# VladimirP1/rs-sync

Hardware: AMD Instinct MI355X
Metric: ray-residuals/sec (PreSync sweep + Sync iter), 4096 frames x 2048 tracks (higher is better)
Workload: dtype f32

## Files before the change

rs-sync_amd/csrc/kernels/support.hpp:

```cpp
#pragma once

namespace {

__global__ __launch_bounds__(64) void plan_sum_kernel(const double* __restrict__ in, uint32_t n_cols,
                                                         const uint32_t* __restrict__ idx,
                                                         const uint32_t* __restrict__ chunk_off, uint32_t n_chunks,
                                                         const uint32_t* __restrict__ win_chunk_off, uint32_t n_win,
                                                         double* __restrict__ chunk_out, double* __restrict__ win_out) {
    const uint32_t r = blockIdx.x / n_win, w = blockIdx.x % n_win;
    const uint32_t c0 = win_chunk_off[w], c1 = win_chunk_off[w + 1];
    const double* row = in + (size_t)r * n_cols;
    double* cout = chunk_out + (size_t)r * n_chunks;
    for (uint32_t c = c0 + threadIdx.x; c < c1; c += blockDim.x) {
        double acc = 0.0;
        uint32_t j = chunk_off[c];
        const uint32_t j1 = chunk_off[c + 1];
        for (; j + 8 <= j1; j += 8) {
            double v[8];
#pragma unroll
            for (int q = 0; q < 8; ++q) v[q] = row[idx ? idx[j + q] : j + q];
#pragma unroll
            for (int q = 0; q < 8; ++q) acc += v[q];
        }
        for (; j < j1; ++j) acc += row[idx ? idx[j] : j];
        cout[c] = acc;
    }
    __syncthreads();
    if (threadIdx.x == 0) {
        double acc = 0.0;
        uint32_t c = c0;
        for (; c + 16 <= c1; c += 16) {
            double v[16];
#pragma unroll
            for (int q = 0; q < 16; ++q) v[q] = cout[c + q];
#pragma unroll
            for (int q = 0; q < 16; ++q) acc += v[q];
        }
        for (; c < c1; ++c) acc += cout[c];
        win_out[blockIdx.x] = acc;
    }
}

struct DebugParams {
    const f4* rays_a;
    const f4* rays_b;
    const FrameRec* frames;
    uint32_t fi;
    const f4* coef;
    int n_knots;
    float fs;
    int32_t kd;
    float fd;
    float* P;
    float* dP;
};

__global__ __launch_bounds__(kBlock) void debug_problem_kernel(DebugParams p) {
    __shared__ f4 s_win[4 * kWinMax];
    const FrameRec fr = p.frames[p.fi];
    Spline sp;
    sp.g = p.coef;
    sp.n = p.n_knots;
    stage_window(sp, s_win, fr.base_knot + (int)floorf(fr.tmin) + p.kd, fr.base_knot + (int)floorf(fr.tmax) + p.kd + 1);
    __syncthreads();
    for (uint32_t row = blockIdx.x * kBlock + threadIdx.x; row < fr.n; row += gridDim.x * kBlock) {
        f3 P, dP;
        if (sp.path == kPathInterior) residual_row<true, kPathInterior>(sp, p.rays_a[fr.off + row], p.rays_b[fr.off + row], fr.base_knot + p.kd, p.fd, P, dP);
        else residual_row<true, kPathGlobal>(sp, p.rays_a[fr.off + row], p.rays_b[fr.off + row], fr.base_knot + p.kd, p.fd, P, dP);
        p.P[3 * row] = P.x; p.P[3 * row + 1] = P.y; p.P[3 * row + 2] = P.z;
        if (p.dP) { p.dP[3 * row] = dP.x * p.fs; p.dP[3 * row + 1] = dP.y * p.fs; p.dP[3 * row + 2] = dP.z * p.fs; }
    }
}

struct PackParams {
    const double* raw;
    const rship_pack_frame* frames;
    f4* rays_a;
    f4* rays_b;
    double2* q0;
    double2* q1;
    double2* q2;
    double2* q3;
    double start, fs;
    uint32_t* bad;
};

__device__ __forceinline__ double pixel_knot_offset(double ro, double py, double frame_time, double rows, double start, double fs,
                                                   double base) {
    return rs::knot_offset(rs::row_time(ro, py, frame_time, rows), start, fs, base);
}

__global__ __launch_bounds__(kBlock) void pack_frames_kernel(PackParams p) {
    const rship_pack_frame& fr = p.frames[blockIdx.x];
    const uint32_t n = fr.n_rays;
    for (uint32_t row = blockIdx.y * kBlock + threadIdx.x; row < n; row += gridDim.y * kBlock) {
        double ra[3], rb[3], tsa, tsb, ta, tb;
        const double* rec = p.raw + fr.raw_offset;
        if (fr.is_pixels) {
            const double2* src = (const double2*)(rec + 4 * (size_t)row);
            const double2 a = src[0], b = src[1];
            const rs::Lens lens{fr.lens[0], fr.lens[1], fr.lens[2], fr.lens[3], fr.lens[4], fr.lens[5], fr.lens[6], fr.lens[7], fr.lens[8]};
            rs::pixel_to_ray(lens, a.x, a.y, fr.time_a, fr.rows, ra, &tsa);
            rs::pixel_to_ray(lens, b.x, b.y, fr.time_b, fr.rows, rb, &tsb);
            ta = pixel_knot_offset(lens.ro, a.y, fr.time_a, fr.rows, p.start, p.fs, fr.base);
            tb = pixel_knot_offset(lens.ro, b.y, fr.time_b, fr.rows, p.start, p.fs, fr.base);
        } else {
            tsa = rec[row];
            tsb = rec[(size_t)n + row];
            const double* pa = rec + 2 * (size_t)n + 3 * (size_t)row;
            const double* pb = rec + 5 * (size_t)n + 3 * (size_t)row;
            ra[0] = pa[0]; ra[1] = pa[1]; ra[2] = pa[2];
            rb[0] = pb[0]; rb[1] = pb[1]; rb[2] = pb[2];
            ta = rs::knot_offset(tsa, p.start, p.fs, fr.base);
            tb = rs::knot_offset(tsb, p.start, p.fs, fr.base);
        }
        f4 o0, o1;
        o0.x = (float)ra[0]; o0.y = (float)rb[0]; o0.z = (float)ra[1]; o0.w = (float)rb[1];
        o1.x = (float)ra[2]; o1.y = (float)rb[2]; o1.z = (float)ta; o1.w = (float)tb;
        const bool ok = finite_f(o0.x) && finite_f(o0.y) && finite_f(o0.z) && finite_f(o0.w) && finite_f(o1.x) &&
                        finite_f(o1.y) && finite_f(o1.z) && finite_f(o1.w);
        if (!ok) atomicAdd(p.bad, 1u);
        const size_t o = (size_t)fr.ray_offset + row;
        p.rays_a[o] = o0;
        p.rays_b[o] = o1;
        p.q0[o] = double2{ra[0], rb[0]};
        p.q1[o] = double2{ra[1], rb[1]};
        p.q2[o] = double2{ra[2], rb[2]};
        p.q3[o] = double2{ta, tb};
    }
}

struct RetimeParams {
    const double* raw;
    const rship_pack_frame* pack;
    const FrameRec* frames;
    const double* ro;
    f4* rays_b;
    double2* q3;
    double start, fs;
};

__global__ __launch_bounds__(kBlock) void retime_pixels_kernel(RetimeParams p) {
    const rship_pack_frame& fr = p.pack[blockIdx.x];
    if (!fr.is_pixels) return;
    const uint32_t n = fr.n_rays;
    const double ro = p.ro[blockIdx.x], base = (double)p.frames[blockIdx.x].base_knot;
    const double* rec = p.raw + fr.raw_offset;
    for (uint32_t row = blockIdx.y * kBlock + threadIdx.x; row < n; row += gridDim.y * kBlock) {
        const double ya = rec[4 * (size_t)row + 1], yb = rec[4 * (size_t)row + 3];
        const double ta = pixel_knot_offset(ro, ya, fr.time_a, fr.rows, p.start, p.fs, base);
        const double tb = pixel_knot_offset(ro, yb, fr.time_b, fr.rows, p.start, p.fs, base);
        const size_t o = (size_t)fr.ray_offset + row;
        ((float2*)(p.rays_b + o))[1] = make_float2((float)ta, (float)tb);
        p.q3[o] = double2{ta, tb};
    }
}

__global__ __launch_bounds__(64) void debug_select_kernel(const float* __restrict__ vals, uint32_t n, uint32_t kq,
                                                          const float* __restrict__ upper, uint32_t* out) {
    constexpr int NR = 32;
    const int lane = threadIdx.x;
    const float* v = vals + (size_t)blockIdx.x * n;
// ... 27 lines not shown
```

rs-sync_amd/csrc/kernels/sync64.hpp:

```cpp
#pragma once

#pragma clang fp contract(off)

namespace {



struct Loss64Params {
    Rays64 rays;
    const FrameRec* frames;
    const uint32_t* sel;
    uint32_t n_sel;
    const d4* coef;
    int n_knots;
    double fs;
    const int32_t* kd;
    const double* fd;
    uint32_t n_delays;
    const uint32_t* grp;
    uint32_t n_grp;
    const double* M;
    const double* k;
    double* part_loss;
    double* part_grad;
// ... 392 lines not shown
    if (fd != fd) {
        if (tid == 0 && p.evals_out) p.evals_out[sf] = 0;
        if (mk_out) { mk_out[0] = m_x; mk_out[1] = m_y; mk_out[2] = m_z; mk_out[3] = m_k; }
        return;
    }

    Spline64 sp;
    sp.g = p.coef;
    sp.n = p.n_knots;
    sp.cap = (int)p.win_cap;
    sp.compact = (int)p.win_compact;
    frame_window64(sp, s_win, fr, kd);
    __syncthreads();

    MotionEval64<RPT, NW, EMU4> ev;
    ev.part = s_part;
    ev.buf = 0;
    ev.evals = 0;
    const int base = fr.base_knot + kd;
    ev.gP = nullptr;
    ev.g_rows = 0;
    ev.rpt = RPT;
    if constexpr (RPT != 0) {
#pragma unroll
        for (int j = 0; j < RPT; ++j) {
            const uint32_t row = j * kThreads + tid;
            d3 P = d3{0, 0, 0}, dP;
            if (row < N) residual_row64<false>(sp, p.rays, (size_t)fr.off + row, base, fd, P, dP);
            ev.P[j] = P;
        }
    } else {
        double* gp = p.scratch + (size_t)scratch_entry * 3 * p.scratch_rows;
        ev.gP = gp;
        ev.g_rows = p.scratch_rows;
        constexpr int kGroup = EMU4 ? 256 : kThreads;
        ev.rpt = (int)((N + kGroup - 1) / kGroup);
        for (uint32_t row = tid; row < (uint32_t)ev.rpt * kGroup; row += kThreads) {
            d3 P = d3{0, 0, 0}, dP;
            if (row < N) residual_row64<false>(sp, p.rays, (size_t)fr.off + row, base, fd, P, dP);
            gp[row] = P.x; gp[p.scratch_rows + row] = P.y; gp[2 * (size_t)p.scratch_rows + row] = P.z;
        }
    }

    double x[3];
    double kk;
    if (p.simple_k || pend != kInitNone) {
        d3 Mv = d3{0, 0, 0};
        if (!p.simple_k && pend >= 0) {
            uint32_t i0, i1;
            rs::sample_pair(p.seed, fr.id, p.win_stream ? ld_m<SC1>(&p.win_stream[grp]) : p.stream_base + grp * p.stream_stride, (uint32_t)pend, N, i0, i1);
            d3 P0, P1, dP;
            residual_row64<false>(sp, p.rays, (size_t)fr.off + i0, base, fd, P0, dP);
            residual_row64<false>(sp, p.rays, (size_t)fr.off + i1, base, fd, P1, dP);
            Mv = rs::cross(P0, P1);
            const double nn = sqrt(rs::dot(Mv, Mv));
            if (!(nn < 1e-12)) Mv = rs::scale(Mv, 1.0 / nn);
        }
        double tot;
        if constexpr (EMU4) {
            tot = 0.0;
            for (int vw = 0; vw < 4; ++vw) {
                double ss = 0.0;
                for (int j = 0; j < ev.rpt; ++j) {
                    const size_t i = (size_t)j * 256 + (size_t)vw * 64 + tid;
                    const d3 Pj = d3{ev.gP[i], ev.gP[ev.g_rows + i], ev.gP[2 * (size_t)ev.g_rows + i]};
                    const double pm = p.simple_k ? sqrt(rs::dot(Pj, Pj)) : rs::dot(Pj, Mv);
                    ss = fma(pm, pm, ss);
                }
                const double sw = wave_sum_f64(ss);
                tot = vw == 0 ? sw : tot + sw;
            }
        } else {
        double ss = 0.0;
        if constexpr (RPT != 0) {
#pragma unroll
            for (int j = 0; j < RPT; ++j) {
                const double pm = p.simple_k ? sqrt(rs::dot(ev.P[j], ev.P[j])) : rs::dot(ev.P[j], Mv);
                ss = fma(pm, pm, ss);
            }
        } else {
            for (int j = 0; j < ev.rpt; ++j) {
                const size_t i = (size_t)j * kThreads + tid;
                const d3 Pj = d3{ev.gP[i], ev.gP[ev.g_rows + i], ev.gP[2 * (size_t)ev.g_rows + i]};
                const double pm = p.simple_k ? sqrt(rs::dot(Pj, Pj)) : rs::dot(Pj, Mv);
                ss = fma(pm, pm, ss);
            }
        }
        const double sw = wave_sum_f64(ss);
        if ((tid & 63) == 0) s_red[tid >> 6] = sw;
        __syncthreads();
        tot = s_red[0];
#pragma unroll
        for (int w = 1; w < NW; ++w) tot += s_red[w];
        }
        kk = clamp_k(100.0 / sqrt(tot));
        x[0] = Mv.x; x[1] = Mv.y; x[2] = Mv.z;
        if (tid == 0) {
            if (!p.simple_k) { st_m<SC1>(&p.M[3 * sf], x[0]); st_m<SC1>(&p.M[3 * sf + 1], x[1]); st_m<SC1>(&p.M[3 * sf + 2], x[2]); }
            st_m<SC1>(&p.k[sf], kk);
            if (p.init_h) st_m<SC1>(&p.init_h[sf], (int32_t)kInitNone);
        }
    } else {
        x[0] = m_x; x[1] = m_y; x[2] = m_z;
        kk = m_k;
    }
    if (mk_out) { mk_out[0] = x[0]; mk_out[1] = x[1]; mk_out[2] = x[2]; mk_out[3] = kk; }
    if (p.max_iters <= 0 || p.simple_k) return;
    ev.k2 = kk * kk;
    if constexpr (EMU4) {
        if ((size_t)N * 24u <= (size_t)p.win_bytes) {
            __syncthreads();
            __attribute__((address_space(3))) double* l = (__attribute__((address_space(3))) double*)reinterpret_cast<double*>(s_win);
            for (uint32_t row = tid; row < N; row += kThreads) {
                l[row] = ev.gP[row];
                l[N + row] = ev.gP[ev.g_rows + row];
                l[2 * N + row] = ev.gP[2 * (size_t)ev.g_rows + row];
            }
            __syncthreads();
            ev.lP = l;
            ev.n_lds = N;
        }
    }

    LbfgsHistLds hist{s_S, s_Y, s_inv_ys, s_rho, s_alpha};
    int best_not_last = 0;
    K3_T0();
    const int it = rs::lbfgs3(ev, hist, x, p.max_iters , p.reeval, &best_not_last);
    K3_ADD(12, 13);
    K3_FLUSH(ev);
    if (mk_out) { mk_out[0] = x[0]; mk_out[1] = x[1]; mk_out[2] = x[2]; }
    if (tid == 0) {
        st_m<SC1>(&p.M[3 * sf], x[0]); st_m<SC1>(&p.M[3 * sf + 1], x[1]); st_m<SC1>(&p.M[3 * sf + 2], x[2]);
        if (p.stats) {
            atomicAdd(&p.stats[0], (unsigned long long)it);
            atomicAdd(&p.stats[1], (unsigned long long)ev.evals);
            atomicAdd(&p.stats[2], (unsigned long long)best_not_last);
        }
        if (p.per_frame) {
            p.per_frame[2 * sf] = (uint32_t)it;
            p.per_frame[2 * sf + 1] = (uint32_t)ev.evals;
        }
        if (p.evals_out) p.evals_out[sf] = (uint32_t)ev.evals;
    }
}

template <int RPT, int NW>
__global__ __launch_bounds__(64 * NW, NW == 4 ? (RPT == 0 ? 2 : (RPT <= 8 ? 3 : (RPT <= 24 ? 2 : 1))) : (NW == 1 ? (RPT >= 8 ? 3 : 4) : 2)) void opt_motion64_kernel(Motion64Params p) {
    __shared__ MotionLds<NW> lds;
    extern __shared__ d4 s_motion_win[];
    opt_motion64_body<RPT, NW>(p, p.order ? p.order[blockIdx.x + p.slot0] : blockIdx.x + p.slot0, lds, s_motion_win, nullptr,
                               p.scratch0 + blockIdx.x);
}

__global__ __launch_bounds__(1024) void motion_order_kernel(const uint32_t* __restrict__ evals, const uint32_t* __restrict__ list,
                                                            uint32_t* __restrict__ order, uint32_t pos0, uint32_t count) {
    __shared__ uint32_t s_bin[256];
    for (uint32_t b = threadIdx.x; b < 256; b += blockDim.x) s_bin[b] = 0;
    __syncthreads();
    for (uint32_t i = threadIdx.x; i < count; i += blockDim.x) {
        const uint32_t e = evals[list[pos0 + i]];
        atomicAdd(&s_bin[e < 255u ? e : 255u], 1u);
    }
    __syncthreads();
    if (threadIdx.x == 0) {
        uint32_t at = 0;
        for (int b = 255; b >= 0; --b) {
            const uint32_t n = s_bin[b];
            s_bin[b] = at;
            at += n;
        }
    }
    __syncthreads();
    for (uint32_t i = threadIdx.x; i < count; i += blockDim.x) {
        const uint32_t s = list[pos0 + i];
        const uint32_t e = evals[s];
        const uint32_t pos = atomicAdd(&s_bin[e < 255u ? e : 255u], 1u);
        order[pos0 + pos] = s;
    }
}

struct Debug64Params {
    Rays64 rays;
    const FrameRec* frames;
    uint32_t fi;
    const d4* coef;
    int n_knots;
    double fs;
    int32_t kd;
    double fd;
    double* P;
    double* dP;
};

__global__ __launch_bounds__(kBlock) void debug_problem64_kernel(Debug64Params p) {
    __shared__ d4 s_win[4 * kWinMax];
    const FrameRec fr = p.frames[p.fi];
    Spline64 sp;
    sp.g = p.coef;
    sp.n = p.n_knots;
    sp.cap = kWinMax;
    sp.compact = 0;
    frame_window64(sp, s_win, fr, p.kd);
    __syncthreads();
    for (uint32_t row = blockIdx.x * kBlock + threadIdx.x; row < fr.n; row += gridDim.x * kBlock) {
        d3 P, dP;
        residual_row64<true>(sp, p.rays, (size_t)fr.off + row, fr.base_knot + p.kd, p.fd, P, dP);
        p.P[3 * row] = P.x; p.P[3 * row + 1] = P.y; p.P[3 * row + 2] = P.z;
        if (p.dP) { p.dP[3 * row] = dP.x * p.fs; p.dP[3 * row + 1] = dP.y * p.fs; p.dP[3 * row + 2] = dP.z * p.fs; }
    }
}

__global__ __launch_bounds__(64) void debug_math64_kernel(int op, const double* __restrict__ a, const double* __restrict__ b,
                                                          double* __restrict__ out, uint32_t n) {
    const uint32_t i = blockIdx.x * 64 + threadIdx.x;
    const double x = i < n ? a[i] : 0.0, y = (i < n && b) ? b[i] : 0.0;
    if (op == 4) {
        const double t = wave_sum_f64(x);
        if (threadIdx.x == 0) out[blockIdx.x] = t;
        return;
    }
    if (i >= n) return;
    if (op == 0) out[i] = x / y;
    else if (op == 1) out[i] = sqrt(x);
    else if (op == 2) { double rc; out[2 * i] = rs::log1p_rcp_f64(x, &rc); out[2 * i + 1] = rc; }
    else if (op == 5) out[i] = rs::div3_exact(x);
    else out[i] = fma(x, y, x);
}

}

#pragma clang fp contract(fast)
```

rs-sync_amd/csrc/kernels/syncloop.hpp:

```cpp
#pragma once

namespace {

constexpr int kMaxBt = 10, kHalfBt = 5;

struct SyncWin {
    double d, v;
    double x0;
    double l1, g1;
    int active, conv, hit, iters;
    int phase;
    int nf;
    int hit_prev;
};

struct SyncLoopParams {
    SyncWin* win;
    uint32_t n_win;
    uint32_t win0, win1;
    const double* part;
    uint32_t n_sel, rows;
    const uint32_t* chunk_off;
    const uint32_t* win_chunk_off;
    double* chunk_tmp;
    uint32_t chunk_stride;
    int32_t* mo_kd; double* mo_fd;
    int32_t* lg_kd; double* lg_fd;
    int32_t* tr_kd; double* tr_fd;
    double fs;
    double ts[11];
    double c_armijo, delay_b, search_center, search_radius;
    int it, max_outer;
    int nf_fixed;
    int nf_floor;
    double* ext_sums;
    int* n_active;
    double* trace;
};


__device__ __forceinline__ void split64_dev(double delay, double fs, int32_t* kd, double* fd) {
#pragma clang fp contract(off)
    if (delay != delay) { *kd = 0; *fd = delay; return; }
    const double D = delay * fs;
    const double kClamp = (double)(1 << 29);
    if (!(fabs(D) <= 1.79769313486231570e308)) { *kd = 0; *fd = 0.0; return; }
    const double fl = floor(D);
    if (fl > kClamp) { *kd = 1 << 29; *fd = 0.0; return; }
    if (fl < -kClamp) { *kd = -(1 << 29); *fd = 0.0; return; }
    *kd = (int32_t)fl;
    *fd = D - fl;
}

constexpr uint32_t kStageDoubles = 2048;
__device__ __forceinline__ void window_sums(const SyncLoopParams& p, uint32_t w, double* s_tot, double* s_stage) {
    const uint32_t c0 = p.win_chunk_off[w], c1 = p.win_chunk_off[w + 1], nc = c1 - c0;
    const uint32_t j_lo = p.chunk_off[c0], j_hi = p.chunk_off[c1], span = j_hi - j_lo;
    double* tmp = p.chunk_tmp + (size_t)w * (2 * kMaxBt) * p.chunk_stride;
    const bool staged = p.rows * span <= kStageDoubles;
    if (staged) {
        for (uint32_t e = threadIdx.x; e < p.rows * span; e += blockDim.x)
            s_stage[e] = p.part[(size_t)(e / span) * p.n_sel + j_lo + e % span];
        __syncthreads();
    }
    for (uint32_t e = threadIdx.x; e < p.rows * nc; e += blockDim.x) {
        const uint32_t r = e / nc, c = c0 + e % nc;
        double acc = 0.0;
        uint32_t j = p.chunk_off[c];
        const uint32_t j1 = p.chunk_off[c + 1];
        if (staged) {
            const double* row = s_stage + (size_t)r * span - j_lo;
            for (; j + 8 <= j1; j += 8) {
                double v[8];
#pragma unroll
                for (int q = 0; q < 8; ++q) v[q] = row[j + q];
#pragma unroll
                for (int q = 0; q < 8; ++q) acc += v[q];
            }
            for (; j < j1; ++j) acc += row[j];
        } else {
            const double* row = p.part + (size_t)r * p.n_sel;
            const uint32_t cnt = j1 - j;
            if (cnt <= 64) {
                double v[64];
#pragma unroll
                for (int q = 0; q < 64; ++q) v[q] = (uint32_t)q < cnt ? row[j + q] : 0.0;
#pragma unroll
                for (int q = 0; q < 64; ++q)
                    if ((uint32_t)q < cnt) acc += v[q];
            } else {
                for (; j < j1; ++j) acc += row[j];
            }
        }
        tmp[(size_t)r * p.chunk_stride + (c - c0)] = acc;
    }
    __syncthreads();
    for (uint32_t r = threadIdx.x; r < p.rows; r += blockDim.x) {
        const double* t = tmp + (size_t)r * p.chunk_stride;
        double acc = 0.0;
        uint32_t c = 0;
        for (; c + 16 <= nc; c += 16) {
            double v[16];
#pragma unroll
            for (int q = 0; q < 16; ++q) v[q] = t[c + q];
#pragma unroll
            for (int q = 0; q < 16; ++q) acc += v[q];
        }
        for (; c < nc; ++c) acc += t[c];
        s_tot[r] = acc;
    }
    __syncthreads();
}

__global__ __launch_bounds__(64) void sync_begin_kernel(SyncLoopParams p) {
#pragma clang fp contract(off)
    const uint32_t w = p.win0 + blockIdx.x * 64 + threadIdx.x;
    if (w >= p.win1) return;
    SyncWin& s = p.win[w];
    s.x0 = s.active ? s.d - p.delay_b * s.v : __builtin_nan("");
    split64_dev(s.active ? s.d : __builtin_nan(""), p.fs, &p.mo_kd[w], &p.mo_fd[w]);
    split64_dev(s.x0, p.fs, &p.lg_kd[w], &p.lg_fd[w]);
}

__device__ __forceinline__ bool trial_wanted(const SyncWin& s, int i) {
    if (!s.active) return false;
    return s.phase == 0 ? i < s.nf : i >= s.nf;
}

__device__ __forceinline__ void grad_decide(const SyncLoopParams& p, SyncWin& s, double l1, double g1) {
#pragma clang fp contract(off)
    if (s.active && s.phase == 0) {
        s.l1 = l1;
        s.g1 = g1;
        s.hit = -1;
        if (s.iters == 0 && !p.nf_fixed) {
            int i = 0;
            while (i < kMaxBt - 1 && p.ts[i] * fabs(s.g1) >= 1e-3) ++i;
            const int want = i + 2;
            s.nf = want < kHalfBt ? kHalfBt : (want > kMaxBt ? kMaxBt : want);
        }
    }
}
__device__ __forceinline__ void trial_delays(const SyncLoopParams& p, const SyncWin& s, int32_t* tr_kd, double* tr_fd, size_t stride) {
#pragma clang fp contract(off)
    for (int i = 0; i < kMaxBt; ++i) {
        const double td = trial_wanted(s, i) ? s.x0 - p.ts[i] * s.g1 : __builtin_nan("");
        split64_dev(td, p.fs, &tr_kd[(size_t)i * stride], &tr_fd[(size_t)i * stride]);
    }
}

__global__ __launch_bounds__(kBlock) void sync_sums_kernel(SyncLoopParams p) {
#pragma clang fp contract(off)
    __shared__ double s_tot[2 * kMaxBt];
    __shared__ double s_stage[kStageDoubles];
    const uint32_t w = blockIdx.x + p.win0;
    window_sums(p, w, s_tot, s_stage);
    for (uint32_t r = threadIdx.x; r < p.rows; r += blockDim.x) p.ext_sums[(size_t)r * p.n_win + w] = s_tot[r];
}
__device__ __forceinline__ void decision_sums(const SyncLoopParams& p, uint32_t w, double* s_tot, double* s_stage) {
    if (p.ext_sums) {
        for (uint32_t r = threadIdx.x; r < p.rows; r += blockDim.x) s_tot[r] = p.ext_sums[(size_t)r * p.n_win + w];
        __syncthreads();
    } else {
        window_sums(p, w, s_tot, s_stage);
    }
}

__global__ __launch_bounds__(kBlock) void sync_grad_kernel(SyncLoopParams p) {
#pragma clang fp contract(off)
    __shared__ double s_tot[2 * kMaxBt];
    __shared__ double s_stage[kStageDoubles];
    const uint32_t w = blockIdx.x + p.win0;
    decision_sums(p, w, s_tot, s_stage);
    if (threadIdx.x != 0) return;
    SyncWin& s = p.win[w];
    grad_decide(p, s, s_tot[0], s_tot[1]);
    trial_delays(p, s, p.tr_kd + w, p.tr_fd + w, p.n_win);
}

__device__ __forceinline__ void armijo(const SyncLoopParams& p, SyncWin& s, const double* lt, int b0, int b1) {
#pragma clang fp contract(off)
    if (!s.active || s.hit >= 0) return;
    const double m = s.g1 * s.g1;
    for (int i = b0; i < b1; ++i) {
        if (s.l1 - lt[i] >= p.ts[i] * p.c_armijo * m) {
            s.hit = i;
            break;
        }
    }
}

__device__ __forceinline__ bool step_decide(const SyncLoopParams& p, SyncWin& s, const double* lt, double* rows, size_t row_stride) {
#pragma clang fp contract(off)
    bool step_now = false;
    if (s.active) {
        if (s.phase == 0) {
            armijo(p, s, lt, 0, s.nf);
            if (s.hit >= 0 || s.nf >= kMaxBt) step_now = true;
            else s.phase = 1;
        } else {
            armijo(p, s, lt, s.nf, kMaxBt);
            step_now = true;
        }
    }
    if (step_now) {
        const double v = s.l1, g = s.g1;
        const double t = s.hit >= 0 ? p.ts[s.hit] : p.ts[kMaxBt];
        const int trials = s.hit >= 0 ? s.hit + 1 : kMaxBt;
        const double step = -t * g;
        s.v = p.delay_b * s.v + step;
        s.d += s.v;
        const double step_size = fabs(step);
        double* row = rows + (size_t)s.iters * row_stride;
        row[0] = s.d; row[1] = step; row[2] = v; row[3] = g; row[4] = t; row[5] = (double)trials;
        s.iters += 1;
        s.phase = 0;
        const int last = s.hit >= 0 ? s.hit : kMaxBt - 1;
        const int want = (last > s.hit_prev ? last : s.hit_prev) + 1;
        s.hit_prev = last;
        s.nf = p.nf_fixed ? p.nf_fixed : (want < p.nf_floor ? p.nf_floor : (want > kMaxBt ? kMaxBt : want));
        if (step_size < 1e-4) s.conv++; else s.conv = 0;
        bool stop = s.conv > 5;
        if (!stop && fabs(s.d - p.search_center) > p.search_radius) stop = true;
        if (stop || s.iters == p.max_outer) s.active = 0;
    }
    s.x0 = s.active ? s.d - p.delay_b * s.v : __builtin_nan("");
    return step_now;
}

__global__ __launch_bounds__(kBlock) void sync_step_kernel(SyncLoopParams p) {
#pragma clang fp contract(off)
    __shared__ double s_tot[2 * kMaxBt];
    __shared__ double s_stage[kStageDoubles];
    const uint32_t w = blockIdx.x + p.win0;
    decision_sums(p, w, s_tot, s_stage);
    if (threadIdx.x != 0) return;
    SyncWin& s = p.win[w];
    step_decide(p, s, s_tot, p.trace + (size_t)w * 6, (size_t)p.n_win * 6);
    if (s.active) atomicAdd(&p.n_active[p.it], 1);
    const bool go = s.active && s.phase == 0;
    split64_dev(go ? s.d : __builtin_nan(""), p.fs, &p.mo_kd[w], &p.mo_fd[w]);
    split64_dev(go ? s.x0 : __builtin_nan(""), p.fs, &p.lg_kd[w], &p.lg_fd[w]);
}

}
```

rs-sync_amd/csrc/rssync_kernels.hip:

```cpp
#include <hip/hip_runtime.h>

#include <dlfcn.h>

#include <algorithm>
#include <cmath>
#include <cstdio>
#include <cstdlib>
#include <cstring>
#include <mutex>
#include <string>
#include <thread>
#include <vector>

#ifndef RSSYNC_TEST_VARIANTS
#define RSSYNC_TEST_VARIANTS 0
#endif

#include "../../include/rssync_hip.h"
#include "track_hip.h"
#include "rectify_hip.h"
#include "stabilize_hip.h"
#include "color_hip.h"
#include "zoom_hip.h"
#include "limit_hip.h"
#include "colorzoom_hip.h"
#include "infill_hip.h"
#include "colorinfill_hip.h"
#include "device_math.hpp"
#include "sync_math.hpp"
#include "lens_math.hpp"
#include "rectify_math.hpp"
#include "stabilize_math.hpp"
#include "color_math.hpp"
#include "resample_math.hpp"
#include "zoom_math.hpp"
#include "limit_math.hpp"
#include "infill_math.hpp"
#include "gyro_math.hpp"
#include "gyro_signal_math.hpp"
#include "window_plan.hpp"
#include "frame_plan.hpp"
#include "roctx_ranges.hpp"

using rs::f3;
using rs::f4;

#include "kernels/common.hpp"
#include "kernels/rows64.hpp"
#include "kernels/lmeds.hpp"
#include "kernels/lmeds_small.hpp"
#include "kernels/lmeds_big.hpp"
#include "kernels/support.hpp"
#include "kernels/sync64.hpp"
#include "kernels/syncloop.hpp"
#include "kernels/exec_big.hpp"
#include "kernels/executor.hpp"
#include "kernels/gyro.hpp"
#include "kernels/track.hpp"
#include "kernels/features.hpp"
#include "kernels/rectify.hpp"
#include "kernels/stabilize.hpp"
#include "kernels/color.hpp"
#include "kernels/color16.hpp"
#include "kernels/resample.hpp"
#include "kernels/zoom.hpp"
#include "kernels/limit.hpp"
#include "kernels/colorzoom.hpp"
#include "kernels/infill.hpp"
#include "kernels/colorinfill.hpp"


struct DevBuf {
    void* p = nullptr;
    size_t cap = 0;
};
struct TempBuf : DevBuf {
    TempBuf() = default;
    TempBuf(const TempBuf&) = delete;
    TempBuf& operator=(const TempBuf&) = delete;
    ~TempBuf() {
        if (p) (void)hipFree(p);
    }
};

constexpr int kNumClasses = 6;

struct rship_ctx {
    int device = 0;
    hipStream_t own_stream = nullptr;
    hipStream_t stream = nullptr;
    hipStream_t copy_stream = nullptr;
    hipEvent_t copy_done = nullptr;
    std::string err;
    DevBuf coef, coef64, raw, rays_a, rays_b, rays64, frames, sel, M, k, grp, grp_off, init_h;
    DevBuf pack_list, retime_ro;
    std::vector<std::vector<char>> retime_staged;
    std::vector<uint32_t> h_ray_off;
    double pack_start = 0, pack_fs = 0;
    DevBuf mo_evals, mo_order;
    std::vector<std::pair<uint32_t, uint32_t>> mo_ranges;
    bool mo_identity = false;
    DevBuf plan_idx, plan_chunk_off, plan_win_off, chunk_out, win_out;
    uint32_t plan_max_chunks = 0;
    DevBuf g_ts, g_rates, g_us, g_dq, g_q, g_knots, g_cf, g_status;
    uint32_t g_n = 0;
    DevBuf gc_a, gc_b, gc_seg, gc_rates;
    bool gc_on = false;
    uint32_t gc_n = 0, gc_k = 1;
    double gc_sr = 0, gc_first = 0;
    double g_first_s = 0, g_last_s = 0;
    DevBuf trk_slot[2], trk_out;
    DevBuf ftr_cells, ftr_out;
    hipEvent_t trk_up[2] = {}, trk_k[2] = {};
    DevBuf rect_rays, rect_slot[2], rect_times, rect_count, rect_tmp;
    double rect_key[10] = {};
    bool rect_rays_ok = false;
    DevBuf stab_weights, stab_targets, stab_zooms, stab_cover;
    DevBuf rect_rays_c;
    DevBuf limit_goal, limit_out, limit_rays;
    double rect_key_c[10] = {};
    bool rect_rays_c_ok = false;
    int64_t g_first_us = 0, g_last_us = 0;
    std::vector<hipStream_t> loop_streams;
    hipEvent_t loop_ready = nullptr;
    std::vector<uint32_t> h_grp_off;
    DevBuf loop_state;
    bool plan_has_idx = false;
    uint32_t plan_chunks = 0, plan_wins = 0, plan_len = 0;
    struct Pend { uint32_t rows = 0; bool grad = false, frame_costs = false, best_h = false; size_t off_chunk = 0, off_flags = 0; } pend;
    bool init_pending = false;
    uint64_t init_seed = 0;
    uint32_t init_stream = 0, init_stride = 0;
    uint32_t n_knots = 0, n_frames = 0, n_sel = 0, max_n = 0, n_grp = 1;
    uint64_t total_rays = 0;
    double fs = 0;
    int lbfgs_reeval = 0;
    DevBuf cls_slots;
    std::vector<uint32_t> h_cls_slots;
    uint32_t cls_off[kNumClasses + 1] = {};
    uint32_t cls_max_n[kNumClasses] = {};
    int cls_used = 0;
    std::vector<rs::FrameDims> own_dims, problem_dims;
    uint32_t cls_cap64[kNumClasses] = {80, 80, 80, 80, 80, 80};
    bool cls_compact = false;
    bool no_compact = false;
    bool force_general = false;
    uint32_t one_wave_max = 512;
    uint32_t exec_big_max = 2048;
    uint32_t exec_big_share = 8;
    bool force_big = false;
    bool no_small_loss = false;
    bool exact_select = false;
    bool no_subshapes = false;
    bool no_small_lmeds = false;
    float max_span = 0.f;
    float max_ends = 0.f;
    int lds_per_cu = 160 * 1024;
    uint32_t last_lmeds_shape[kNumClasses] = {};
    uint32_t last_lmeds_cap = 0, last_lmeds_chunk = 0, last_init_cap = 0;
    void* rccl_lib = nullptr;
    std::string rccl_path;
    void* rccl_comm = nullptr;
    DevBuf rccl_buf;
    DevBuf big_scratch, mo_scratch;
    rship_loop_exchange_fn loop_xchg = nullptr;
    void* loop_xchg_user = nullptr;
    uint64_t loop_exchanges = 0;
    uint32_t exec_last[4] = {0, 0, 0, 0};
    std::vector<uint32_t> h_frame_n;
    std::vector<uint32_t> h_sel;
    std::vector<uint32_t> h_delays, h_delays64;
    const float* d_fd = nullptr;
    DevBuf kd64;
    const double* d_fd64 = nullptr;
    DevBuf redo_mask, redo_delays, redo_count, init_delays64;
    bool no_fp64_rows = false;
    bool redo_dirty = true;
    uint64_t near_launches = 0;
    struct PendRedo { bool armed = false; LmedsParams p{}; double step_knots = 0; uint32_t chunk = 1; bool uploaded = false; } pend_redo;
    std::vector<int32_t> h_kd64r;
    std::vector<double> h_fd64r;
    std::vector<uint32_t> h_init64;
    uint32_t batch_n = 0, batch_next = 0, batch_rows = 0;
    size_t batch_chunk_stride = 0, batch_win_stride = 0;
    DevBuf dump, dump_ncont;
    bool dump_on = false;
    uint32_t dump_rows = 0, dump_dims[4] = {0, 0, 0, 0}, dump_ncont_n = 0;
    DevBuf kd, frame_cost, best_h, costs, part, flags, stats;
    void* pinned = nullptr;
    size_t pinned_cap = 0;
    bool prof = false;
    struct Pending { int kind; hipEvent_t a, b; };
    std::vector<Pending> pending;
    std::vector<hipEvent_t> pool;
    uint64_t launches[RSHIP_K_COUNT] = {};
    double total_ms[RSHIP_K_COUNT] = {};
};

namespace {

std::mutex g_err_mutex;
int set_err(rship_ctx* c, const char* what, hipError_t e) {
    std::lock_guard<std::mutex> lock(g_err_mutex);
    c->err = std::string(what) + ": " + hipGetErrorString(e);
    return 1;
}
int set_err(rship_ctx* c, const std::string& what) {
    std::lock_guard<std::mutex> lock(g_err_mutex);
    c->err = what;
    return 1;
}

#define RS_HIP(call)                                         \
    do {                                                     \
        hipError_t e__ = (call);                             \
        if (e__ != hipSuccess) return set_err(c, #call, e__); \
    } while (0)

int ensure(rship_ctx* c, DevBuf& b, size_t bytes) {
    if (bytes <= b.cap) return 0;
    if (b.p) RS_HIP(hipFree(b.p));
    b.p = nullptr;
    b.cap = 0;
    size_t want = bytes + bytes / 4 + 256;
    RS_HIP(hipMalloc(&b.p, want));
    b.cap = want;
    return 0;
}

int ensure_pinned(rship_ctx* c, size_t bytes) {
    if (bytes <= c->pinned_cap) return 0;
    if (c->pinned) RS_HIP(hipHostFree(c->pinned));
    c->pinned = nullptr;
    c->pinned_cap = 0;
    size_t want = bytes + bytes / 4 + 4096;
    RS_HIP(hipHostMalloc(&c->pinned, want, hipHostMallocDefault));
    c->pinned_cap = want;
    return 0;
}

const char* const kKindNames[RSHIP_K_COUNT] = {"rssync:K2 lmeds sweep", "rssync:K1 loss (trials)", "rssync:K3 motion L-BFGS", "rssync:window sums",
                                               "rssync:K2 GuessMotion search", "rssync:pack frames", "rssync:gyro pipeline", "rssync:K1 loss+gradient",
                                               "rssync:retime pixels"};
struct ProfScope {
    rship_ctx* c;
    int kind;
    hipEvent_t a = nullptr, b = nullptr;
    rs::RoctxRange range;
    ProfScope(rship_ctx* c_, int kind_) : c(c_), kind(kind_), range(kKindNames[kind_]) {
        if (!c->prof) return;
        auto get = [&]() {
            hipEvent_t e = nullptr;
            if (!c->pool.empty()) { e = c->pool.back(); c->pool.pop_back(); }
            else (void)hipEventCreate(&e);
            return e;
        };
        a = get();
        b = get();
        (void)hipEventRecord(a, c->stream);
    }
    ~ProfScope() {
        if (!c->prof) return;
        (void)hipEventRecord(b, c->stream);
        c->pending.push_back({kind, a, b});
    }
};

void prof_collect(rship_ctx* c) {
    for (auto& pd : c->pending) {
        float ms = 0.f;
        if (hipEventElapsedTime(&ms, pd.a, pd.b) == hipSuccess) {
            c->launches[pd.kind] += 1;
            c->total_ms[pd.kind] += (double)ms;
        }
        c->pool.push_back(pd.a);
        c->pool.push_back(pd.b);
    }
    c->pending.clear();
}

int sync_stream(rship_ctx* c) {
    RS_HIP(hipStreamSynchronize(c->stream));
    prof_collect(c);
    c->retime_staged.clear();
    return 0;
}

constexpr int kMaxRpt = 32;
constexpr int kFourWaveMaxRpt = 24;
constexpr int kWideBlock = 512;

static_assert(rs::kPlanBlock == (uint32_t)kBlock && rs::kPlanFourWaveMaxRpt == (uint32_t)kFourWaveMaxRpt && rs::kPlanMaxRpt == (uint32_t)kMaxRpt,
              "window_plan.hpp (the rules, checked on the CPU by tests/test_window_plan.py) and this file disagree on the size classes");
int class_of(const rship_ctx* c, uint32_t n) {
    if (c->force_big) return 5;
    return rs::plan_class_of(n, c->one_wave_max);
}
void class_bounds(const rship_ctx* c, int k, uint32_t* lo, uint32_t* hi) {
    if (c->force_big) { *lo = k == 5 ? 0u : 1u; *hi = k == 5 ? 0xffffffffu : 0u; return; }
    const uint32_t top[6] = {c->one_wave_max, 4u * kBlock, 8u * kBlock, (uint32_t)kFourWaveMaxRpt * kBlock, (uint32_t)kMaxRpt * kBlock, 0xffffffffu};
    *hi = top[k];
    *lo = k == 0 ? 0u : top[k - 1] + 1u;
}
int class_rpt(const rship_ctx* c, int k) { return rs::plan_class_shape(k, c->cls_max_n[k]); }
int small_rpt(uint32_t n_all) { return rs::plan_small_rows(n_all, false); }
int rpt_for(uint32_t max_n) {
    if (max_n > (uint32_t)kMaxRpt * kBlock) return 0;
    int rpt = 4;
    while ((uint32_t)rpt * kBlock < max_n) rpt *= 2;
    return rpt;
}
uint32_t big_rows(uint32_t max_n) { return (max_n + kBlock - 1) / kBlock * kBlock; }

const std::vector<rs::FrameDims>& plan_dims(const rship_ctx* c) { return c->problem_dims.empty() ? c->own_dims : c->problem_dims; }
void update_class_caps(rship_ctx* c) {
    const std::vector<rs::FrameDims>& d = plan_dims(c);
    for (int k = 0; k < kNumClasses; ++k) {
        uint32_t lo, hi;
        class_bounds(c, k, &lo, &hi);
        bool comp = false;
        const bool may_compact = k == 0 && !c->no_compact && !c->no_small_loss && !c->force_general;
        c->cls_cap64[k] = c->force_general ? (uint32_t)rs::kPlanWinStatic : rs::cap64_frames(d.data(), d.size(), lo, hi, k == 0, may_compact ? &comp : nullptr);
        if (k == 0) c->cls_compact = comp;
    }
}

struct ClassRange {
    int k;
    uint32_t pos0, count;
    const uint32_t* list;
};
std::vector<ClassRange> class_ranges(const rship_ctx* c, uint32_t slot0 = 0, uint32_t count = 0) {
    std::vector<ClassRange> out;
    if (!count) { slot0 = 0; count = c->n_sel; }
    const uint32_t* L = c->h_cls_slots.data();
    for (int k = 0; k < kNumClasses; ++k) {
        const uint32_t* a = L + c->cls_off[k];
        const uint32_t* b = L + c->cls_off[k + 1];
        if (a == b) continue;
        const uint32_t* lo = std::lower_bound(a, b, slot0);
        const uint32_t* hi = std::lower_bound(a, b, slot0 + count);
        if (lo == hi) continue;
        const uint32_t pos0 = (uint32_t)(lo - L);
        out.push_back(ClassRange{k, pos0, (uint32_t)(hi - lo), c->cls_used > 1 ? (const uint32_t*)c->cls_slots.p + pos0 : nullptr});
    }
    return out;
}
int main_class(const rship_ctx* c) {
    int best = 0;
    uint32_t most = 0;
    for (int k = 0; k < kNumClasses; ++k) {
        const uint32_t n = c->cls_off[k + 1] - c->cls_off[k];
        if (n > most) { most = n; best = k; }
    }
    if (!most) {
        uint32_t mx = 0;
        for (const rs::FrameDims& d : c->own_dims) mx = std::max(mx, d.n);
        best = class_of(c, mx);
    }
    return best;
}

constexpr uint32_t kLossWinBytes = kLossBatch * kWinMax * 128u;
using rs::WinPlan;
static_assert(rs::kPlanWinStatic == (uint32_t)kWinMax, "window_plan.hpp and kernels/common.hpp disagree on the compiled-in window");
uint32_t cap64_of(const rship_ctx* c, int k) { return c->cls_cap64[k]; }
bool compact_of(const rship_ctx* c, int k) { return k == 0 && c->cls_compact; }
size_t win64_bytes(const rship_ctx* c, int k) { return (size_t)c->cls_cap64[k] * (compact_of(c, k) ? 64u : 128u); }
float class_span(const rship_ctx* c, int k) {
    uint32_t lo, hi;
    class_bounds(c, k, &lo, &hi);
    float m = 0.f;
    for (const rs::FrameDims& d : plan_dims(c))
        if (d.n && d.n >= lo && d.n <= hi) m = std::max(m, d.span);
    return m;
}
template <class K>
uint32_t static_lds_of(K kernel) {
    hipFuncAttributes a{};
    if (hipFuncGetAttributes(&a, reinterpret_cast<const void*>(kernel)) != hipSuccess) { (void)hipGetLastError(); return 0; }
    return (uint32_t)a.sharedSizeBytes;
}
template <class K>
void allow_dynamic_lds(K kernel, size_t bytes) {
    if (bytes > 32 * 1024) {
        (void)hipFuncSetAttribute(reinterpret_cast<const void*>(kernel), hipFuncAttributeMaxDynamicSharedMemorySize, (int)bytes);
        (void)hipGetLastError();
    }
}

// ... 170 lines not shown
    if (wp.cap) {
        if (rpt == 16 && wp.extra_wg) {
            allow_dynamic_lds(lmeds_kernel<16, MODE, 1>, dyn);
            hipLaunchKernelGGL((lmeds_kernel<16, MODE, 1>), dim3(grid), dim3(kBlock), dyn, c->stream, p);
        } else if (!with_tile_shape<MODE>(rpt, [&](auto sh) {
                       constexpr int R = decltype(sh)::rpt, B = decltype(sh)::block;
                       allow_dynamic_lds(lmeds_kernel<R, MODE, 0, true, false, B>, dyn);
                       hipLaunchKernelGGL((lmeds_kernel<R, MODE, 0, true, false, B>), dim3(grid), dim3(B), dyn, c->stream, p);
                   })) {
            return set_err(c, "lmeds: unsupported rows-per-thread");
        }
        RS_HIP(hipGetLastError());
        return 0;
    }
#if RSSYNC_TEST_VARIANTS
    if (MODE == 0 && c->exact_select) {
        switch (rpt) {
            case 4: hipLaunchKernelGGL((lmeds_kernel<4, 0, kWinMax, false>), dim3(grid), dim3(kBlock), 0, c->stream, p); break;
            case 8: hipLaunchKernelGGL((lmeds_kernel<8, 0, kWinMax, false>), dim3(grid), dim3(kBlock), 0, c->stream, p); break;
            case 16: hipLaunchKernelGGL((lmeds_kernel<16, 0, kWinMax, false>), dim3(grid), dim3(kBlock), 0, c->stream, p); break;
            case 24: allow_dynamic_lds(lmeds_kernel<24, 0, kWinMax, false>, 0);
                     hipLaunchKernelGGL((lmeds_kernel<24, 0, kWinMax, false>), dim3(grid), dim3(kBlock), 0, c->stream, p); break;
            case 32: hipLaunchKernelGGL((lmeds_kernel<16, 0, kWinMax, false, false, kWideBlock>), dim3(grid), dim3(kWideBlock), 0, c->stream, p); break;
            default: return set_err(c, "lmeds: unsupported rows-per-thread");
        }
        RS_HIP(hipGetLastError());
        return 0;
    }
#endif
    if (!with_tile_shape<MODE>(rpt, [&](auto sh) {
            constexpr int R = decltype(sh)::rpt, B = decltype(sh)::block;
            if (B != kBlock || R > 16) allow_dynamic_lds(lmeds_kernel<R, MODE, kWinMax, true, false, B>, 0);
            hipLaunchKernelGGL((lmeds_kernel<R, MODE, kWinMax, true, false, B>), dim3(grid), dim3(B), 0, c->stream, p);
        }))
        return set_err(c, "lmeds: unsupported rows-per-thread");
    RS_HIP(hipGetLastError());
    return 0;
}

template <int MODE>
int launch_lmeds(rship_ctx* c, const LmedsParams& p, double step_knots, uint32_t chunk_want, uint32_t* main_cap, uint32_t* main_chunk) {
    ProfScope ps(c, MODE == 1 ? RSHIP_K_INIT : RSHIP_K_LMEDS);
    const int mk = main_class(c);
    if (MODE == 0) memset(c->last_lmeds_shape, 0, sizeof(c->last_lmeds_shape));
    for (const ClassRange& r : class_ranges(c)) {
        const WinPlan wp = plan_lmeds_window<MODE>(c, r.k, step_knots, chunk_want);
        if (r.k == mk) {
            if (main_cap) *main_cap = wp.cap;
            if (main_chunk) *main_chunk = wp.chunk;
        }
        if (launch_lmeds_class<MODE>(c, p, r, wp)) return 1;
    }
    return 0;
}

int ensure_redo_count(rship_ctx* c) {
    if (c->redo_count.p) return 0;
    if (ensure(c, c->redo_count, 16)) return 1;
    RS_HIP(hipMemsetAsync(c->redo_count.p, 0, 16, c->stream));
    return 0;
}

int launch_lmeds_redo(rship_ctx* c, const LmedsParams& p_in, double step_knots, uint32_t chunk_want) {
    ProfScope ps(c, RSHIP_K_LMEDS);
    for (const ClassRange& r : class_ranges(c)) {
        const LmedsKind kind = lmeds_kind(c, r.k);
        if (kind == LmedsKind::Big) continue;
        const WinPlan wp = plan_lmeds_window<0>(c, r.k, step_knots, chunk_want);
        const int rpt = lmeds_rpt(c, r.k);
        LmedsParams p = p_in;
        p.slots = r.list;
        p.n_slots = r.count;
        p.chunk = wp.chunk;
        p.n_chunks = (p.n_cand + wp.chunk - 1) / wp.chunk;
        if (kind == LmedsKind::Small) {
            const uint32_t g1 = (uint32_t)((uint64_t)r.count * p.n_chunks);
            switch (rpt) {
                case 1: hipLaunchKernelGGL((lmeds_small_kernel<1, 0, 0, true>), dim3(g1), dim3(64), 0, c->stream, p); break;
                case 2: hipLaunchKernelGGL((lmeds_small_kernel<2, 0, 0, true>), dim3(g1), dim3(64), 0, c->stream, p); break;
                case 3: hipLaunchKernelGGL((lmeds_small_kernel<3, 0, 0, true>), dim3(g1), dim3(64), 0, c->stream, p); break;
                case 4: hipLaunchKernelGGL((lmeds_small_kernel<4, 0, 0, true>), dim3(g1), dim3(64), 0, c->stream, p); break;
                default: hipLaunchKernelGGL((lmeds_small_kernel<8, 0, 0, true>), dim3(g1), dim3(64), 0, c->stream, p); break;
            }
        } else {
            const uint32_t grid = (uint32_t)((uint64_t)((r.count + 7) / 8) * 8 * p.n_chunks);
            switch (rpt) {
                case 4: hipLaunchKernelGGL((lmeds_kernel<4, 0, 0, true, true>), dim3(grid), dim3(kBlock), 0, c->stream, p); break;
                case 8: hipLaunchKernelGGL((lmeds_kernel<8, 0, 0, true, true>), dim3(grid), dim3(kBlock), 0, c->stream, p); break;
                case 16: hipLaunchKernelGGL((lmeds_kernel<16, 0, 0, true, true>), dim3(grid), dim3(kBlock), 0, c->stream, p); break;
                case 24: allow_dynamic_lds(lmeds_kernel<24, 0, 0, true, true>, 0);
                         hipLaunchKernelGGL((lmeds_kernel<24, 0, 0, true, true>), dim3(grid), dim3(kBlock), 0, c->stream, p); break;
                case 32: allow_dynamic_lds(lmeds_kernel<16, 0, 0, true, true, kWideBlock>, 0);
                         hipLaunchKernelGGL((lmeds_kernel<16, 0, 0, true, true, kWideBlock>), dim3(grid), dim3(kWideBlock), 0, c->stream, p); break;
                default: return set_err(c, "lmeds (fp64 rows): unsupported rows-per-thread");
            }
        }
        RS_HIP(hipGetLastError());
    }
    return 0;
}

bool loss_fixed80(const rship_ctx* c, int k) {
    return c->cls_cap64[k] == (uint32_t)kWinMax && (class_span(c, k) + 1.f <= (float)kWinMax || c->force_general);
}
uint32_t loss_nb_run(const rship_ctx* c, int k) {
    return loss_fixed80(c, k) ? (uint32_t)kLossBatch : std::max(1u, std::min((uint32_t)kLossBatchWide, kLossWinBytes / (c->cls_cap64[k] * 128u)));
}

template <bool GRAD, bool SIMPLE>
int launch_loss64(rship_ctx* c, const Loss64Params& p_in, hipStream_t st = nullptr, uint32_t slot0 = 0, uint32_t count = 0) {
    if (!st) st = c->stream;
    ProfScope ps(c, GRAD ? RSHIP_K_LOSS_GRAD : RSHIP_K_LOSS);
    for (const ClassRange& r : class_ranges(c, slot0, count)) {
        Loss64Params p = p_in;
        const int k = r.k;
        p.slots = r.list;
        p.slot0 = r.list ? 0u : c->h_cls_slots[r.pos0];
        const uint32_t cap64 = cap64_of(c, k);
        p.win_cap = cap64;
        p.win_compact = compact_of(c, k) ? 1u : 0u;
        const bool fixed80 = !GRAD && loss_fixed80(c, k);
        p.nb_run = GRAD ? 1u : loss_nb_run(c, k);
        const size_t dyn = fixed80 ? 0 : (size_t)p.nb_run * cap64 * 128u, dyn_small = win64_bytes(c, k);
        if (k == 0 && !c->no_small_loss) {
            hipLaunchKernelGGL((loss64_small_kernel<GRAD, SIMPLE>), dim3(r.count), dim3(64), dyn_small, st, p);
            RS_HIP(hipGetLastError());
            continue;
        }
        const int rpt = k == 0 ? rpt_for(c->cls_max_n[0]) : class_rpt(c, k);
#define RS_LOSS_CASE(R)                                                                                                        \
    case R:                                                                                                                    \
        if constexpr (!GRAD) {                                                                                                 \
            if (fixed80) { hipLaunchKernelGGL((loss64_kernel<R, GRAD, SIMPLE, kWinMax>), dim3(r.count), dim3(kBlock), 0, st, p); break; } \
        }                                                                                                                      \
        hipLaunchKernelGGL((loss64_kernel<R, GRAD, SIMPLE, 0>), dim3(r.count), dim3(kBlock), dyn, st, p);                      \
        break;
        switch (rpt) {
            RS_LOSS_CASE(0)
            RS_LOSS_CASE(4)
            RS_LOSS_CASE(8)
            RS_LOSS_CASE(16)
            RS_LOSS_CASE(24)
            RS_LOSS_CASE(32)
            default: return set_err(c, "loss: unsupported rows-per-thread");
        }
#undef RS_LOSS_CASE
        RS_HIP(hipGetLastError());
    }
    return 0;
}

constexpr uint32_t kOrderMinSlots = 512;

int launch_motion64(rship_ctx* c, const Motion64Params& p_in, hipStream_t st = nullptr, uint32_t slot0 = 0, uint32_t count = 0) {
    if (!st) st = c->stream;
    ProfScope ps(c, RSHIP_K_MOTION);
    for (const ClassRange& r : class_ranges(c, slot0, count)) {
        Motion64Params p = p_in;
        const int k = r.k;
        p.slot0 = r.pos0;
        p.win_cap = cap64_of(c, k);
        p.win_compact = compact_of(c, k) ? 1u : 0u;
        const size_t dyn = win64_bytes(c, k);
        p.win_bytes = (uint32_t)dyn;
        const uint32_t cnt = r.count;
        if (k == 0) {
            const uint32_t n = c->cls_max_n[0];
            if (n <= 64) hipLaunchKernelGGL((opt_motion64_kernel<1, 1>), dim3(cnt), dim3(64), dyn, st, p);
            else if (n <= 128) hipLaunchKernelGGL((opt_motion64_kernel<2, 1>), dim3(cnt), dim3(64), dyn, st, p);
            else if (n <= 192) hipLaunchKernelGGL((opt_motion64_kernel<3, 1>), dim3(cnt), dim3(64), dyn, st, p);
            else if (n <= 256) hipLaunchKernelGGL((opt_motion64_kernel<4, 1>), dim3(cnt), dim3(64), dyn, st, p);
            else hipLaunchKernelGGL((opt_motion64_kernel<8, 1>), dim3(cnt), dim3(64), dyn, st, p);
        } else if (k == 1) hipLaunchKernelGGL((opt_motion64_kernel<4, 4>), dim3(cnt), dim3(256), dyn, st, p);
        else if (k == 2) hipLaunchKernelGGL((opt_motion64_kernel<8, 4>), dim3(cnt), dim3(256), dyn, st, p);
        else if (k == 3 && class_rpt(c, 3) == 16) hipLaunchKernelGGL((opt_motion64_kernel<16, 4>), dim3(cnt), dim3(256), dyn, st, p);
        else if (k == 3) hipLaunchKernelGGL((opt_motion64_kernel<24, 4>), dim3(cnt), dim3(256), dyn, st, p);
        else if (k == 4) hipLaunchKernelGGL((opt_motion64_kernel<32, 4>), dim3(cnt), dim3(256), dyn, st, p);
        else {
            if (!p.scratch || p.scratch_rows < c->cls_max_n[5]) return set_err(c, "motion: no scratch for frames of more than 8192 tracks");
            p.scratch0 = r.pos0 - c->cls_off[5];
            hipLaunchKernelGGL((opt_motion64_kernel<0, 4>), dim3(cnt), dim3(256), dyn, st, p);
        }
        RS_HIP(hipGetLastError());
        if (p.evals_out && p.order && c->mo_order.p && p.max_iters > 0 && !p.simple_k && cnt >= kOrderMinSlots) {
            hipLaunchKernelGGL(motion_order_kernel, dim3(1), dim3(1024), 0, st, (const uint32_t*)p.evals_out, (const uint32_t*)c->cls_slots.p,
                               (uint32_t*)c->mo_order.p, r.pos0, cnt);
            RS_HIP(hipGetLastError());
        }
    }
    return 0;
}

int launch_plan_sum(rship_ctx* c, const double* in, uint32_t rows, uint32_t cols, uint32_t slot = 0, uint32_t n_slots = 1) {
    if (!c->plan_wins) return set_err(c, "no reduction plan set");
    const size_t cs = (size_t)rows * (c->plan_chunks + 1), ws = (size_t)rows * c->plan_wins;
    if (n_slots > 1 && (c->chunk_out.cap < cs * n_slots * 8 || c->win_out.cap < ws * n_slots * 8)) return set_err(c, "plan sum: the batch's buffers were not sized");
    if (n_slots == 1 && (ensure(c, c->chunk_out, cs * 8) || ensure(c, c->win_out, ws * 8))) return 1;
    ProfScope ps(c, RSHIP_K_REDUCE);
    hipLaunchKernelGGL(plan_sum_kernel, dim3(rows * c->plan_wins), dim3(64), 0, c->stream, in, cols,
                       c->plan_has_idx ? (const uint32_t*)c->plan_idx.p : nullptr, (const uint32_t*)c->plan_chunk_off.p,
                       c->plan_chunks, (const uint32_t*)c->plan_win_off.p, c->plan_wins, (double*)c->chunk_out.p + cs * slot,
                       (double*)c->win_out.p + ws * slot);
    RS_HIP(hipGetLastError());
    return 0;
}

int queue_sums_to_host(rship_ctx* c, uint32_t rows, size_t at, size_t* off_chunk, size_t* end) {
    const size_t wb = (size_t)rows * c->plan_wins * 8, cb = (size_t)rows * c->plan_chunks * 8;
    if (ensure_pinned(c, at + wb + cb + 64)) return 1;
    RS_HIP(hipMemcpyAsync((char*)c->pinned + at, c->win_out.p, wb, hipMemcpyDeviceToHost, c->stream));
    if (cb) RS_HIP(hipMemcpyAsync((char*)c->pinned + at + wb, c->chunk_out.p, cb, hipMemcpyDeviceToHost, c->stream));
    *off_chunk = at + wb;
    *end = at + wb + cb;
    return 0;
}

struct DeviceGuard {
    int prev = -1;
    explicit DeviceGuard(const rship_ctx* c) {
        if (hipGetDevice(&prev) != hipSuccess) prev = -1;
        if (prev != c->device) (void)hipSetDevice(c->device);
        else prev = -1;
    }
    ~DeviceGuard() {
        if (prev >= 0) (void)hipSetDevice(prev);
    }
    DeviceGuard(const DeviceGuard&) = delete;
    DeviceGuard& operator=(const DeviceGuard&) = delete;
};

int upload_delays(rship_ctx* c, const int32_t* kd, const float* fd, size_t n) {
    if (ensure(c, c->kd, n * 8)) return 1;
    c->h_delays.resize(2 * n);
    memcpy(c->h_delays.data(), kd, n * 4);
    memcpy(c->h_delays.data() + n, fd, n * 4);
    RS_HIP(hipMemcpyAsync(c->kd.p, c->h_delays.data(), n * 8, hipMemcpyHostToDevice, c->stream));
    c->d_fd = (const float*)((const int32_t*)c->kd.p + n);
    return 0;
}
int upload_delays64(rship_ctx* c, const int32_t* kd, const double* fd, size_t n) {
    const size_t pad = (n + 1) / 2 * 2;
    if (ensure(c, c->kd64, pad * 4 + n * 8)) return 1;
    c->h_delays64.resize(pad + 2 * n);
    memcpy(c->h_delays64.data(), kd, n * 4);
    memcpy(c->h_delays64.data() + pad, fd, n * 8);
    RS_HIP(hipMemcpyAsync(c->kd64.p, c->h_delays64.data(), pad * 4 + n * 8, hipMemcpyHostToDevice, c->stream));
    c->d_fd64 = (const double*)((const int32_t*)c->kd64.p + pad);
    return 0;
}
Rays64 rays64_of(const rship_ctx* c) {
    const double2* q0 = (const double2*)c->rays64.p;
    const size_t tr = (size_t)c->total_rays;
    return Rays64{q0, q0 + tr, q0 + 2 * tr, q0 + 3 * tr};
}
int check_ready(rship_ctx* c) {
    if (!c->n_knots) return set_err(c, "no gyro spline uploaded");
    if (!c->n_frames) return set_err(c, "no frames uploaded");
    if (!c->n_sel) return set_err(c, "no frames selected");
    return 0;
}

}

namespace {
struct RcclId { char bytes[128]; };
using rccl_get_id_fn = int (*)(RcclId*);
using rccl_init_fn = int (*)(void**, int, RcclId, int);
using rccl_allreduce_fn = int (*)(const void*, void*, size_t, int, int, void*, hipStream_t);
using rccl_destroy_fn = int (*)(void*);

using rccl_abort_fn = int (*)(void*);

void* rccl_sym(rship_ctx* c, const char* name) {
    if (!c->rccl_lib) {
        Dl_info info{};
        std::string dir, hip_path;
        if (dladdr(reinterpret_cast<const void*>(&hipStreamSynchronize), &info) && info.dli_fname) {
            hip_path = info.dli_fname;
            const size_t cut = hip_path.rfind('/');
            if (cut != std::string::npos) dir = hip_path.substr(0, cut + 1);
        }
        std::vector<std::string> tries;
        if (!dir.empty()) { tries.push_back(dir + "librccl.so.1"); tries.push_back(dir + "librccl.so"); }
        for (const char* lib : {"librccl.so.1", "librccl.so", "/opt/rocm/lib/librccl.so.1"}) tries.push_back(lib);
        for (size_t i = 0; i < tries.size() && !c->rccl_lib; ++i) {
            c->rccl_lib = dlopen(tries[i].c_str(), RTLD_NOW | RTLD_LOCAL);
            if (c->rccl_lib)
                c->rccl_path = tries[i] + (i < 2 && !dir.empty() ? " (beside the HIP runtime this library is bound to, " + hip_path + ")"
                                                                 : " (opened by name)");
        }
        if (!c->rccl_lib) {
            set_err(c, std::string("rccl: cannot open librccl: ") + dlerror());
            return nullptr;
        }
    }
    void* f = dlsym(c->rccl_lib, name);
    if (!f) set_err(c, std::string("rccl: missing symbol ") + name);
    return f;
}

void rccl_abort_comm(rship_ctx* c) {
    if (!c->rccl_comm) return;
    std::string keep;
    { std::lock_guard<std::mutex> lock(g_err_mutex); keep = c->err; }
    if (auto ab = (rccl_abort_fn)rccl_sym(c, "ncclCommAbort")) (void)ab(c->rccl_comm);
    c->rccl_comm = nullptr;
    set_err(c, keep + " -- the RCCL communicator was aborted so that the other ranks fail instead of waiting");
}
}

extern "C" {

int rship_max_tracks(void) { return 1 << 24; }
int rship_has_device_loop(void) { return 1; }

void* rship_host_alloc(size_t bytes) {
    void* p = nullptr;
    if (hipHostMalloc(&p, bytes ? bytes : 1, hipHostMallocDefault) == hipSuccess && p) return p;
    (void)hipGetLastError();
    return nullptr;
}
void rship_host_free(void* p) {
    if (p) (void)hipHostFree(p);
}

int rship_create(rship_ctx** out, int device) {
    *out = nullptr;
    int ndev = 0;
    hipError_t e = hipGetDeviceCount(&ndev);
    if (e != hipSuccess || ndev == 0) return 2;
    rship_ctx* c = new rship_ctx();
    if (const char* s = std::getenv("RSSYNC_NO_SMALL_LMEDS")) c->no_small_lmeds = s[0] && s[0] != '0';
    if (const char* s = std::getenv("RSSYNC_NO_SUBSHAPES")) c->no_subshapes = s[0] && s[0] != '0';
    if (const char* s = std::getenv("RSSYNC_K2_EXACT_SELECT")) c->exact_select = s[0] && s[0] != '0';
#if !RSSYNC_TEST_VARIANTS
    if (c->exact_select) {
        fprintf(stderr, "rssync: RSSYNC_K2_EXACT_SELECT needs the test-variants build (tools/k2_build_variant.sh testvariants -DRSSYNC_TEST_VARIANTS=1)\n");
        delete c;
        return 5;
    }
#endif
    if (const char* s = std::getenv("RSSYNC_NO_SMALL_LOSS")) c->no_small_loss = s[0] && s[0] != '0';
    if (const char* s = std::getenv("RSSYNC_FORCE_BIG")) c->force_big = s[0] && s[0] != '0';
    if (const char* s = std::getenv("RSSYNC_FORCE_GENERAL_SPLINE")) c->force_general = s[0] && s[0] != '0';
    if (const char* s = std::getenv("RSSYNC_NO_COMPACT_WINDOW")) c->no_compact = s[0] && s[0] != '0';
    if (const char* s = std::getenv("RSSYNC_NO_FP64_ROWS")) c->no_fp64_rows = s[0] && s[0] != '0';
    if (const char* s = std::getenv("RSSYNC_EXEC_BIG_MAX")) { const int v = atoi(s); if (v >= 0) c->exec_big_max = (uint32_t)v; }
    if (const char* s = std::getenv("RSSYNC_EXEC_BIG_SHARE")) { const int v = atoi(s); if (v >= 1) c->exec_big_share = (uint32_t)v; }
    if (const char* s = std::getenv("RSSYNC_ONE_WAVE_MAX")) { const int v = atoi(s); if (v >= 64 && v <= 64 * kSmallMaxRpt) c->one_wave_max = (uint32_t)v; }
    if (device >= 0) {
        e = hipSetDevice(device);
        if (e != hipSuccess) { delete c; return 3; }
        c->device = device;
    } else {
        (void)hipGetDevice(&c->device);
    }
    e = hipStreamCreateWithFlags(&c->own_stream, hipStreamNonBlocking);
    if (e == hipSuccess) e = hipStreamCreateWithFlags(&c->copy_stream, hipStreamNonBlocking);
    if (e == hipSuccess) e = hipEventCreateWithFlags(&c->copy_done, hipEventDisableTiming);
    if (e != hipSuccess) { delete c; return 4; }
    c->stream = c->own_stream;
    {
        int v = 0;
        if (hipDeviceGetAttribute(&v, hipDeviceAttributeMaxSharedMemoryPerMultiprocessor, c->device) == hipSuccess && v >= 64 * 1024) c->lds_per_cu = v;
        else (void)hipGetLastError();
    }
    *out = c;
    return 0;
}

void rship_destroy(rship_ctx* c) {
    if (!c) return;
    DeviceGuard dev_guard(c);
    (void)hipStreamSynchronize(c->stream);
    prof_collect(c);
    if (c->rccl_comm) {
        if (auto destroy = (rccl_destroy_fn)rccl_sym(c, "ncclCommDestroy")) (void)destroy(c->rccl_comm);
    }
    if (c->rccl_buf.p) (void)hipFree(c->rccl_buf.p);
    for (auto e : c->pool) (void)hipEventDestroy(e);
    if (c->copy_stream) (void)hipStreamSynchronize(c->copy_stream);
    DevBuf* bufs[] = {&c->pack_list, &c->retime_ro, &c->coef, &c->coef64, &c->raw, &c->rays_a, &c->rays_b, &c->rays64, &c->frames, &c->sel, &c->M, &c->k, &c->grp, &c->grp_off,
                      &c->plan_idx, &c->plan_chunk_off, &c->plan_win_off, &c->chunk_out, &c->win_out, &c->loop_state, &c->kd, &c->kd64, &c->init_h,
                      &c->frame_cost, &c->best_h, &c->costs, &c->part, &c->flags, &c->stats, &c->redo_mask, &c->redo_delays, &c->redo_count, &c->init_delays64, &c->dump, &c->dump_ncont,
                      &c->big_scratch, &c->mo_scratch, &c->mo_evals, &c->mo_order,
                      &c->g_ts, &c->g_rates, &c->g_us, &c->g_dq, &c->g_q, &c->g_knots, &c->g_cf, &c->g_status,
                      &c->trk_slot[0], &c->trk_slot[1], &c->trk_out, &c->ftr_cells, &c->ftr_out,
                      &c->rect_rays, &c->rect_slot[0], &c->rect_slot[1], &c->rect_times, &c->rect_count, &c->rect_tmp,
                      &c->stab_weights, &c->stab_targets, &c->stab_zooms, &c->stab_cover, &c->rect_rays_c,
                      &c->limit_goal, &c->limit_out, &c->limit_rays};
    for (DevBuf* b : bufs)
        if (b->p) (void)hipFree(b->p);
    if (c->pinned) (void)hipHostFree(c->pinned);
    for (hipStream_t st : c->loop_streams) (void)hipStreamDestroy(st);
    if (c->loop_ready) (void)hipEventDestroy(c->loop_ready);
    if (c->copy_done) (void)hipEventDestroy(c->copy_done);
    for (hipEvent_t e : {c->trk_up[0], c->trk_up[1], c->trk_k[0], c->trk_k[1]})
        if (e) (void)hipEventDestroy(e);
    if (c->copy_stream) (void)hipStreamDestroy(c->copy_stream);
    if (c->own_stream) (void)hipStreamDestroy(c->own_stream);
    delete c;
}

const char* rship_last_error(const rship_ctx* c) { return c ? c->err.c_str() : "null context"; }

int rship_set_option(rship_ctx* c, int option, int value) {
    switch (option) {
        case RSHIP_OPT_LBFGS_REEVAL: c->lbfgs_reeval = value != 0; return 0;
        case RSHIP_OPT_TRACKS_HINT: return 0;
        default: return set_err(c, "set_option: unknown option");
    }
}

int rship_set_stream(rship_ctx* c, void* hip_stream) {
    DeviceGuard dev_guard(c);
    RS_HIP(hipStreamSynchronize(c->stream));
    c->stream = hip_stream ? (hipStream_t)hip_stream : c->own_stream;
    return 0;
}

namespace {

constexpr uint32_t kMaxKnots = rs::kMaxKnots;

const rs::SplinePivots* spline_pivots() {
    static const rs::SplinePivots t = [] {
        rs::SplinePivots p;
        p.cp[0] = 0.0;
        for (int i = 1; i < rs::kSplinePivots; ++i) p.cp[i] = rs::spline_next_pivot(p.cp[i - 1]);
        return p;
    }();
    return &t;
}

int spline_from_knots(rship_ctx* c, uint32_t n, double sample_rate) {
    if (n < 2) return set_err(c, "spline: need >= 2 knots");
    if (n > kMaxKnots) return set_err(c, "spline: too many knots");
    const rs::SplinePivots& piv = *spline_pivots();
    if (rs::spline_next_pivot(piv.cp[rs::kSplinePivots - 1]) != piv.cp[rs::kSplinePivots - 1])
        return set_err(c, "spline: pivots not stationary");
    const size_t n16 = (size_t)n * 16;
    if (ensure(c, c->coef64, n16 * 8) || ensure(c, c->coef, n16 * 4) || ensure(c, c->g_cf, (size_t)n * 32)) return 1;
    SplineParams p{};
    p.knots = (const double*)c->g_knots.p;
    p.cf = (double*)c->g_cf.p;
    p.coef64 = (double*)c->coef64.p;
    p.coef32 = (float*)c->coef.p;
    p.n = n;
    p.piv = piv;
    const uint32_t threads = ((n + kSplineRun - 1) / kSplineRun) * 4;
    {
        ProfScope ps(c, RSHIP_K_GYRO);
        hipLaunchKernelGGL(spline_forward_kernel, dim3((threads + 255) / 256), dim3(256), 0, c->stream, p);
        hipLaunchKernelGGL(spline_finish_kernel, dim3((threads + 255) / 256), dim3(256), 0, c->stream, p);
    }
    RS_HIP(hipGetLastError());
    c->n_knots = n;
    c->fs = sample_rate;
    return 0;
}

int gyro_status_to_result(rship_ctx* c, const GyroStatus* h, int grid_status, const int64_t* d_ts, rship_gyro_result* out) {
    out->status = RSHIP_GYRO_OK;
    if (h->bad_input) out->status = RSHIP_GYRO_BAD_INPUT;
    else if (grid_status == RSHIP_GYRO_BAD_RATE || grid_status == RSHIP_GYRO_TOO_LARGE) out->status = grid_status;
    else if (h->out_of_order != kNoIndex) {
        int64_t pair[2];
        out->status = RSHIP_GYRO_OUT_OF_ORDER;
        out->bad_pos = h->out_of_order;
        RS_HIP(hipMemcpy(pair, d_ts + (h->out_of_order - 1), 16, hipMemcpyDeviceToHost));
        out->bad_a = pair[0];
        out->bad_b = pair[1];
    } else if (grid_status != RSHIP_GYRO_OK) out->status = grid_status;
    else if (h->bad_knot) out->status = RSHIP_GYRO_BAD_KNOT;
    else if (!std::isfinite(out->fs)) out->status = RSHIP_GYRO_BAD_RATE;
    else if (!std::isfinite(out->start)) out->status = RSHIP_GYRO_BAD_START;
    return 0;
}

int resample_and_solve(rship_ctx* c, const int64_t* d_ts, const double* d_quats, uint32_t n, int64_t first, int64_t last,
                       rship_gyro_result* out, uint32_t status_slot = 0, bool wait = true) {
    const int grid_status = rs::grid_of(first, last, n, kMaxKnots, out);
    GyroStatus* st = (GyroStatus*)c->g_status.p + status_slot;
    const bool have_grid = grid_status == RSHIP_GYRO_OK;
    if (have_grid) {
        if (ensure(c, c->g_knots, (size_t)out->n_knots * 32)) return 1;
        GyroResampleParams p{};
        p.ts = d_ts; p.quats = d_quats; p.knots = (double*)c->g_knots.p; p.st = st;
        p.n = n; p.m = out->n_knots; p.first_sample = out->first_sample; p.sr_hz = (uint64_t)out->fs;
        {
            ProfScope ps(c, RSHIP_K_GYRO);
            hipLaunchKernelGGL(gyro_resample_kernel, dim3((p.m + 255) / 256), dim3(256), 0, c->stream, p);
        }
        RS_HIP(hipGetLastError());
        if (spline_from_knots(c, out->n_knots, out->fs)) return 1;
    }
    if (!wait) {
        out->status = grid_status == RSHIP_GYRO_OK ? RSHIP_GYRO_OK : grid_status;
        return 0;
    }
    if (ensure_pinned(c, 64)) return 1;
    GyroStatus* h = (GyroStatus*)c->pinned;
    RS_HIP(hipMemcpyAsync(h, st, sizeof(GyroStatus), hipMemcpyDeviceToHost, c->stream));
    if (sync_stream(c)) return 1;
    const GyroStatus hs = *h;
    if (gyro_status_to_result(c, &hs, grid_status, d_ts, out)) return 1;
    if (out->status != RSHIP_GYRO_OK) c->n_knots = 0;
    return 0;
}

}

int rship_gyro_uniform(rship_ctx* c, const double* quats, uint32_t n, double sample_rate) {
    DeviceGuard dev_guard(c);
    if (n < 2) return set_err(c, "spline: need >= 2 knots");
    if (n > kMaxKnots) return set_err(c, "spline: too many knots");
    if (ensure(c, c->g_knots, (size_t)n * 32)) return 1;
    RS_HIP(hipMemcpyAsync(c->g_knots.p, quats, (size_t)n * 32, hipMemcpyHostToDevice, c->stream));
    if (spline_from_knots(c, n, sample_rate)) return 1;
    return sync_stream(c);
}

int rship_gyro_timestamped(rship_ctx* c, const int64_t* ts_us, const double* quats, uint32_t n, rship_gyro_result* out) {
    DeviceGuard dev_guard(c);
    if (n < 2) return set_err(c, "gyro: need >= 2 samples");
    if (ensure(c, c->g_us, (size_t)n * 8) || ensure(c, c->g_q, (size_t)n * 32) || ensure(c, c->g_status, sizeof(GyroStatus) * 256)) return 1;
    RS_HIP(hipMemcpyAsync(c->g_us.p, ts_us, (size_t)n * 8, hipMemcpyHostToDevice, c->stream));
    RS_HIP(hipMemcpyAsync(c->g_q.p, quats, (size_t)n * 32, hipMemcpyHostToDevice, c->stream));
    {
        ProfScope ps(c, RSHIP_K_GYRO);
        hipLaunchKernelGGL(gyro_status_reset_kernel, dim3(1), dim3(1), 0, c->stream, (GyroStatus*)c->g_status.p);
        hipLaunchKernelGGL(gyro_order_kernel, dim3((n + 255) / 256), dim3(256), 0, c->stream, (const int64_t*)c->g_us.p,
                           (const double*)c->g_q.p, n, (GyroStatus*)c->g_status.p);
    }
    RS_HIP(hipGetLastError());
    return resample_and_solve(c, (const int64_t*)c->g_us.p, (const double*)c->g_q.p, n, ts_us[0], ts_us[n - 1], out);
}

int rship_gyro_rates_upload(rship_ctx* c, const double* ts_s, const double* rates, uint32_t n) {
    DeviceGuard dev_guard(c);
    if (n < 2) return set_err(c, "gyro: need >= 2 samples");
    if (ensure(c, c->g_ts, (size_t)n * 8) || ensure(c, c->g_rates, (size_t)n * 24)) return 1;
    RS_HIP(hipMemcpyAsync(c->g_ts.p, ts_s, (size_t)n * 8, hipMemcpyHostToDevice, c->stream));
    RS_HIP(hipMemcpyAsync(c->g_rates.p, rates, (size_t)n * 24, hipMemcpyHostToDevice, c->stream));
    RS_HIP(hipStreamSynchronize(c->stream));
    c->g_n = n;
// ... 244 lines not shown
    c->max_span = 0.f;
    c->max_ends = 0.f;
    c->own_dims.assign(n_frames, rs::FrameDims{0u, 0.f, 0.f});
    for (uint32_t i = 0; i < n_frames; ++i) {
        const float span = rs::frame_span(table[i].tmin, table[i].tmax);
        if (table[i].n_rays && span > c->max_span) c->max_span = span;
        const float ends = c->force_general ? span : rs::frame_ends(table[i].range_a, table[i].range_b, span);
        if (table[i].n_rays && ends > c->max_ends) c->max_ends = ends;
        c->own_dims[i] = rs::FrameDims{table[i].n_rays, span, ends};
    }
    update_class_caps(c);
    if (n_frames && c->force_general) {
        std::vector<rship_frame> legacy(table, table + n_frames);
        for (rship_frame& r : legacy) r.range_a = r.range_b = RSHIP_NO_SPLIT;
        c->max_ends = c->max_span;
        if (stable) RS_HIP(hipStreamSynchronize(c->stream));
        RS_HIP(hipMemcpy(c->frames.p, legacy.data(), (size_t)n_frames * sizeof(rship_frame), hipMemcpyHostToDevice));
    } else if (n_frames) {
        RS_HIP(hipMemcpyAsync(c->frames.p, table, (size_t)n_frames * sizeof(rship_frame), hipMemcpyHostToDevice, c->stream));
    }
    return 0;
}

int rship_pack_frames(rship_ctx* c, const rship_frame* table, const rship_pack_frame* pack, uint32_t n_frames,
                      uint64_t total_rays, double start, double fs, uint32_t* bad) {
    DeviceGuard dev_guard(c);
    if (bad) *bad = 0;
    c->n_frames = 0;
    c->n_sel = 0;
    c->h_sel.clear();
    c->h_frame_n.assign(n_frames, 0);
    c->h_ray_off.assign(n_frames, 0);
    c->problem_dims.clear();
    memset(c->cls_off, 0, sizeof(c->cls_off));
    memset(c->cls_max_n, 0, sizeof(c->cls_max_n));
    c->cls_used = 0;
    c->h_cls_slots.clear();
    uint32_t max_n = 0;
    for (uint32_t i = 0; i < n_frames; ++i) {
        if ((uint64_t)table[i].ray_offset + table[i].n_rays > total_rays) return set_err(c, "frame table exceeds ray buffer");
        if (table[i].n_rays != pack[i].n_rays || table[i].ray_offset != pack[i].ray_offset)
            return set_err(c, "pack list does not match the frame table");
        const uint64_t rec = (uint64_t)pack[i].n_rays * (pack[i].is_pixels ? 4 : 8);
        if ((pack[i].raw_offset + rec) * 8 > c->raw.cap && rec) return set_err(c, "pack: record outside the uploaded raw data");
        if (table[i].n_rays > (uint32_t)rship_max_tracks())
            return set_err(c, "frame has more tracks than the kernels accept (" + std::to_string(rship_max_tracks()) + ")");
        c->h_frame_n[i] = table[i].n_rays;
        c->h_ray_off[i] = table[i].ray_offset;
        max_n = std::max(max_n, table[i].n_rays);
    }
    const size_t tr = (size_t)total_rays;
    if (ensure(c, c->rays_a, tr ? tr * 16 : 16) || ensure(c, c->rays_b, tr ? tr * 16 : 16) ||
        ensure(c, c->rays64, tr ? tr * 64 : 64))
        return 1;
    if (ensure(c, c->frames, (size_t)n_frames * sizeof(rship_frame) + 64)) return 1;
    c->total_rays = total_rays;
    if (install_frame_table(c, table, n_frames, false)) return 1;
    uint32_t nb = 0;
    if (n_frames && max_n) {
        DevBuf& dpk = c->pack_list;
        TempBuf dbad;
        if (ensure(c, dpk, (size_t)n_frames * sizeof(rship_pack_frame)) || ensure(c, dbad, 16)) return 1;
        hipError_t e = hipMemcpyAsync(dpk.p, pack, (size_t)n_frames * sizeof(rship_pack_frame), hipMemcpyHostToDevice, c->stream);
        if (e == hipSuccess) e = hipMemsetAsync(dbad.p, 0, 16, c->stream);
        if (e == hipSuccess) e = hipEventRecord(c->copy_done, c->copy_stream);
        if (e == hipSuccess) e = hipStreamWaitEvent(c->stream, c->copy_done, 0);
        if (e == hipSuccess) {
            PackParams p{};
            p.raw = (const double*)c->raw.p;
            p.frames = (const rship_pack_frame*)dpk.p;
            p.rays_a = (f4*)c->rays_a.p;
            p.rays_b = (f4*)c->rays_b.p;
            p.q0 = (double2*)c->rays64.p;
            p.q1 = p.q0 + tr;
            p.q2 = p.q1 + tr;
            p.q3 = p.q2 + tr;
            p.start = start;
            p.fs = fs;
            p.bad = (uint32_t*)dbad.p;
            {
                ProfScope ps(c, RSHIP_K_PIXELS);
                hipLaunchKernelGGL(pack_frames_kernel, dim3(n_frames, (max_n + kBlock - 1) / kBlock), dim3(kBlock), 0, c->stream, p);
            }
            e = hipGetLastError();
        }
        if (e == hipSuccess) e = hipMemcpyAsync(&nb, dbad.p, 4, hipMemcpyDeviceToHost, c->stream);
        if (e == hipSuccess) e = hipStreamSynchronize(c->stream);
        prof_collect(c);
        if (e != hipSuccess) return set_err(c, "pack_frames", e);
    } else {
        RS_HIP(hipStreamSynchronize(c->stream));
    }
    if (bad) *bad = nb;
    c->n_frames = n_frames;
    c->pack_start = start;
    c->pack_fs = fs;
    return 0;
}

int rship_retime_pixels(rship_ctx* c, const rship_frame* table, const double* ro, uint32_t n_frames) {
    DeviceGuard dev_guard(c);
    if (n_frames != c->n_frames) return set_err(c, "retime: the table must have the frames of the last rship_pack_frames");
    for (uint32_t i = 0; i < n_frames; ++i) {
        if (table[i].n_rays != c->h_frame_n[i] || table[i].ray_offset != c->h_ray_off[i])
            return set_err(c, "retime: the table must have the frames of the last rship_pack_frames");
        if (!std::isfinite(ro[i])) return set_err(c, "retime: non-finite readout");
    }
    if (!n_frames) return 0;
    c->retime_staged.emplace_back((size_t)n_frames * (sizeof(rship_frame) + 8));
    char* stage = c->retime_staged.back().data();
    std::memcpy(stage, table, (size_t)n_frames * sizeof(rship_frame));
    std::memcpy(stage + (size_t)n_frames * sizeof(rship_frame), ro, (size_t)n_frames * 8);
    if (install_frame_table(c, (const rship_frame*)stage, n_frames, true)) return 1;
    uint32_t max_n = 0;
    for (uint32_t i = 0; i < n_frames; ++i) max_n = std::max(max_n, c->h_frame_n[i]);
    if (!max_n) return 0;
    if (!c->pack_list.p) return set_err(c, "retime: no packed frames");
    if (ensure(c, c->retime_ro, (size_t)n_frames * 8)) return 1;
    RS_HIP(hipMemcpyAsync(c->retime_ro.p, stage + (size_t)n_frames * sizeof(rship_frame), (size_t)n_frames * 8, hipMemcpyHostToDevice, c->stream));
    RetimeParams p{};
    p.raw = (const double*)c->raw.p;
    p.pack = (const rship_pack_frame*)c->pack_list.p;
    p.frames = (const FrameRec*)c->frames.p;
    p.ro = (const double*)c->retime_ro.p;
    p.rays_b = (f4*)c->rays_b.p;
    p.q3 = (double2*)c->rays64.p + 3 * (size_t)c->total_rays;
    p.start = c->pack_start;
    p.fs = c->pack_fs;
    {
        ProfScope ps(c, RSHIP_K_RETIME);
        hipLaunchKernelGGL(retime_pixels_kernel, dim3(n_frames, (max_n + kBlock - 1) / kBlock), dim3(kBlock), 0, c->stream, p);
    }
    RS_HIP(hipGetLastError());
    return 0;
}

int rship_set_problem_frames(rship_ctx* c, const rship_frame* table_all, uint32_t n_all) {
    c->problem_dims.assign(n_all, rs::FrameDims{0u, 0.f, 0.f});
    for (uint32_t i = 0; i < n_all; ++i) {
        const float span = rs::frame_span(table_all[i].tmin, table_all[i].tmax);
        const float ends = c->force_general ? span : rs::frame_ends(table_all[i].range_a, table_all[i].range_b, span);
        c->problem_dims[i] = rs::FrameDims{table_all[i].n_rays, span, ends};
    }
    update_class_caps(c);
    return 0;
}

int rship_select_slots(rship_ctx* c, const uint32_t* idx, uint32_t n, const uint32_t* grp_off, uint32_t n_grp) {
    DeviceGuard dev_guard(c);
    for (uint32_t i = 0; i < n; ++i)
        if (idx[i] >= c->n_frames) return set_err(c, "select: frame index out of range");
    if (n_grp < 1) n_grp = 1;
    if (grp_off && (grp_off[0] != 0 || grp_off[n_grp] != n)) return set_err(c, "select: bad group offsets");
    if (ensure(c, c->sel, (size_t)n * 4 + 4) || ensure(c, c->grp, (size_t)n * 4 + 4) ||
        ensure(c, c->grp_off, (size_t)(n_grp + 1) * 4))
        return 1;
    if (ensure(c, c->M, (size_t)n * 24 + 24) || ensure(c, c->k, (size_t)n * 8 + 8) || ensure(c, c->init_h, (size_t)n * 4 + 4)) return 1;
    if (ensure(c, c->mo_evals, (size_t)n * 4 + 4) || ensure(c, c->mo_order, (size_t)n * 4 + 4)) return 1;
    c->init_pending = false;
    std::vector<uint32_t> g(n, 0), off(n_grp + 1, 0);
    if (grp_off) {
        off.assign(grp_off, grp_off + n_grp + 1);
        for (uint32_t w = 0; w < n_grp; ++w)
            for (uint32_t j = off[w]; j < off[w + 1]; ++j) g[j] = w;
    } else {
        off[n_grp] = n;
    }
    if (n) {
        RS_HIP(hipMemcpyAsync(c->sel.p, idx, (size_t)n * 4, hipMemcpyHostToDevice, c->stream));
        RS_HIP(hipMemcpyAsync(c->grp.p, g.data(), (size_t)n * 4, hipMemcpyHostToDevice, c->stream));
    }
    RS_HIP(hipMemcpyAsync(c->grp_off.p, off.data(), (size_t)(n_grp + 1) * 4, hipMemcpyHostToDevice, c->stream));
    RS_HIP(hipMemsetAsync(c->M.p, 0, (size_t)n * 24 + 24, c->stream));
    RS_HIP(hipMemsetAsync(c->k.p, 0, (size_t)n * 8 + 8, c->stream));
    RS_HIP(hipMemsetD32Async((hipDeviceptr_t)c->init_h.p, kInitNone, (size_t)n + 1, c->stream));
    {
        std::vector<uint32_t> cnt(kNumClasses + 1, 0);
        uint32_t mx[kNumClasses] = {};
        for (uint32_t i = 0; i < n; ++i) {
            const uint32_t fn = c->h_frame_n[idx[i]];
            const int k = class_of(c, fn);
            cnt[k + 1] += 1;
            mx[k] = std::max(mx[k], fn);
        }
        c->cls_used = 0;
        for (int k = 0; k < kNumClasses; ++k) {
            if (cnt[k + 1]) c->cls_used += 1;
            c->cls_max_n[k] = mx[k];
            c->cls_off[k] = cnt[k];
            cnt[k + 1] += cnt[k];
        }
        c->cls_off[kNumClasses] = n;
        c->h_cls_slots.assign((size_t)n + 1, n);
        uint32_t at[kNumClasses];
        for (int k = 0; k < kNumClasses; ++k) at[k] = c->cls_off[k];
        for (uint32_t i = 0; i < n; ++i) c->h_cls_slots[at[class_of(c, c->h_frame_n[idx[i]])]++] = i;
        if (ensure(c, c->cls_slots, (size_t)n * 4 + 4)) return 1;
        RS_HIP(hipMemcpyAsync(c->cls_slots.p, c->h_cls_slots.data(), (size_t)(n + 1) * 4, hipMemcpyHostToDevice, c->stream));
        RS_HIP(hipMemcpyAsync(c->mo_order.p, c->h_cls_slots.data(), (size_t)(n + 1) * 4, hipMemcpyHostToDevice, c->stream));
        RS_HIP(hipMemsetAsync(c->mo_evals.p, 0, (size_t)n * 4 + 4, c->stream));
        c->mo_identity = true;
        c->mo_ranges.clear();
    }
    RS_HIP(hipStreamSynchronize(c->stream));
    c->h_sel.assign(idx, idx + n);
    c->h_grp_off = off;
    c->n_sel = n;
    c->n_grp = n_grp;
    c->max_n = 0;
    for (int k = 0; k < kNumClasses; ++k) c->max_n = std::max(c->max_n, c->cls_max_n[k]);
    return 0;
}

int rship_select_frames(rship_ctx* c, const uint32_t* idx, uint32_t n) { return rship_select_slots(c, idx, n, nullptr, 1); }

int rship_set_plan(rship_ctx* c, const uint32_t* plan_idx, uint32_t plan_len, const uint32_t* chunk_off, uint32_t n_chunks,
                   const uint32_t* win_chunk_off, uint32_t n_win) {
    DeviceGuard dev_guard(c);
    if (n_win < 1) return set_err(c, "plan: no window");
    if (win_chunk_off[0] != 0 || win_chunk_off[n_win] != n_chunks) return set_err(c, "plan: bad window offsets");
    if (n_chunks && (chunk_off[0] != 0 || chunk_off[n_chunks] != plan_len)) return set_err(c, "plan: bad chunk offsets");
    for (uint32_t j = 0; plan_idx && j < plan_len; ++j)
        if (plan_idx[j] >= c->n_sel) return set_err(c, "plan: slot out of range");
    if (!plan_idx && plan_len > c->n_sel) return set_err(c, "plan: slot out of range");
    if (ensure(c, c->plan_idx, (size_t)plan_len * 4 + 4) || ensure(c, c->plan_chunk_off, (size_t)(n_chunks + 1) * 4) ||
        ensure(c, c->plan_win_off, (size_t)(n_win + 1) * 4))
        return 1;
    if (plan_idx && plan_len) RS_HIP(hipMemcpyAsync(c->plan_idx.p, plan_idx, (size_t)plan_len * 4, hipMemcpyHostToDevice, c->stream));
    const uint32_t zero = 0;
    RS_HIP(hipMemcpyAsync(c->plan_chunk_off.p, n_chunks ? chunk_off : &zero, (size_t)(n_chunks + 1) * 4, hipMemcpyHostToDevice, c->stream));
    RS_HIP(hipMemcpyAsync(c->plan_win_off.p, win_chunk_off, (size_t)(n_win + 1) * 4, hipMemcpyHostToDevice, c->stream));
    RS_HIP(hipStreamSynchronize(c->stream));
    c->plan_has_idx = plan_idx != nullptr;
    c->plan_max_chunks = 0;
    for (uint32_t w = 0; w < n_win; ++w) c->plan_max_chunks = std::max(c->plan_max_chunks, win_chunk_off[w + 1] - win_chunk_off[w]);
    c->plan_chunks = n_chunks;
    c->plan_wins = n_win;
    c->plan_len = plan_len;
    return 0;
}

int rship_presync_enqueue(rship_ctx* c, const int32_t* kd, const float* fd, const int32_t* kd64, const double* fd64, uint32_t n_cand, uint32_t n_hyp,
                          uint32_t stream_base, uint64_t seed, int want_frame_costs, int want_best_h) {
    DeviceGuard dev_guard(c);
    c->pend = rship_ctx::Pend{};
    c->pend_redo = rship_ctx::PendRedo{};
    if (!c->n_knots) return set_err(c, "no gyro spline uploaded");
    if (c->n_grp != 1) return set_err(c, "presync: the selection must not be grouped");
    const uint32_t ns = c->n_sel;
    const uint32_t bn = c->batch_n ? c->batch_n : 1u, bslot = c->batch_n ? c->batch_next : 0u;
    if (c->batch_n) {
        if (bslot >= bn) return set_err(c, "presync: more sweeps than the batch was opened for");
        if (n_cand != c->batch_rows) return set_err(c, "presync: every sweep of a batch has the same candidates");
        if (want_frame_costs || want_best_h) return set_err(c, "presync: no per-frame outputs inside a batch");
        c->batch_next += 1;
    }
    if (!n_cand || !ns) return 0;
    if (ensure(c, c->frame_cost, (size_t)n_cand * ns * 8)) return 1;
    if (want_best_h && ensure(c, c->best_h, (size_t)n_cand * ns * 4)) return 1;
    if (ensure(c, c->flags, 16 + 4 * (size_t)bn)) return 1;
    if (bslot == 0) {
        if (upload_delays(c, kd, fd, n_cand)) return 1;
        RS_HIP(hipMemsetAsync(c->flags.p, 0, 16 + 4 * (size_t)bn, c->stream));
        if (c->batch_n) {
            if (!c->plan_wins) return set_err(c, "no reduction plan set");
            if (ensure(c, c->chunk_out, (size_t)bn * n_cand * (c->plan_chunks + 1) * 8) || ensure(c, c->win_out, (size_t)bn * n_cand * c->plan_wins * 8)) return 1;
        }
    }

    LmedsParams p{};
    p.rays_a = (const f4*)c->rays_a.p;
    p.rays_b = (const f4*)c->rays_b.p;
    p.frames = (const FrameRec*)c->frames.p;
    p.sel = (const uint32_t*)c->sel.p;
    p.n_sel = ns;
    p.coef = (const f4*)c->coef.p;
    p.n_knots = (int)c->n_knots;
    p.kd = (const int32_t*)c->kd.p;
    p.fd = c->d_fd;
    p.n_cand = n_cand;
    p.grp = nullptr;
    p.n_grp = 1;
    uint64_t work = (uint64_t)n_cand * ns;
    uint32_t chunk = (uint32_t)(work / 8192);
    if (chunk < 1) chunk = 1;
    if (chunk > (uint32_t)kMaxChunk) chunk = kMaxChunk;
    if (chunk > n_cand) chunk = n_cand;
    double step_knots = 0.0;
    if (n_cand > 1) step_knots = std::fabs(((double)kd[n_cand - 1] + fd[n_cand - 1] - (double)kd[0] - fd[0]) / (double)(n_cand - 1));
    p.n_hyp = n_hyp;
    p.stream_base = stream_base;
    p.seed = seed;
    p.frame_cost = (double*)c->frame_cost.p;
    p.best_h = want_best_h ? (int32_t*)c->best_h.p : nullptr;
    p.flags = (uint32_t*)c->flags.p + bslot;
    if (!c->no_fp64_rows && c->rays64.p && c->coef64.p) {
        const uint32_t words = (n_cand + 31u) / 32u;
        const size_t mask_bytes = (size_t)ns * words * 4;
        const void* before = c->redo_mask.p;
        if (ensure(c, c->redo_mask, mask_bytes) || ensure_redo_count(c)) return 1;
        if (c->redo_mask.p != before || c->redo_dirty) {
            RS_HIP(hipMemsetAsync(c->redo_mask.p, 0, c->redo_mask.cap, c->stream));
            c->redo_dirty = false;
        }
        c->h_kd64r.assign(n_cand, 0);
        c->h_fd64r.assign(n_cand, 0.0);
        for (uint32_t i = 0; i < n_cand; ++i) {
            c->h_kd64r[i] = kd64 ? kd64[i] : kd[i];
            c->h_fd64r[i] = fd64 ? fd64[i] : (double)fd[i];
        }
        p.redo_mask = (uint32_t*)c->redo_mask.p;
        p.mask_words = words;
        p.src64 = Rows64Src{rays64_of(c), (const d4*)c->coef64.p, (int)c->n_knots};
        p.redo_count = (unsigned long long*)c->redo_count.p;
        c->pend_redo.uploaded = false;
        if (c->cls_off[5] != c->cls_off[6]) {
            const size_t pad = (n_cand + 1) / 2 * 2;
            if (ensure(c, c->redo_delays, pad * 4 + (size_t)n_cand * 8)) return 1;
            RS_HIP(hipMemcpyAsync(c->redo_delays.p, c->h_kd64r.data(), (size_t)n_cand * 4, hipMemcpyHostToDevice, c->stream));
            RS_HIP(hipMemcpyAsync((char*)c->redo_delays.p + pad * 4, c->h_fd64r.data(), (size_t)n_cand * 8, hipMemcpyHostToDevice, c->stream));
            c->pend_redo.uploaded = true;
            p.kd64 = (const int32_t*)c->redo_delays.p;
            p.fd64 = (const double*)((const char*)c->redo_delays.p + pad * 4);
        }
        c->pend_redo.armed = true;
        c->pend_redo.step_knots = step_knots;
        c->pend_redo.chunk = chunk;
    }
    if (c->dump_on) {
        const uint64_t words = (uint64_t)n_cand * ns * n_hyp * c->dump_rows;
        if (words > ((uint64_t)3 << 30) / 4) return set_err(c, "debug_residuals: more than 3 GB of residuals: sweep fewer candidates per call");
        if (ensure(c, c->dump, (size_t)words * 4)) return 1;
        RS_HIP(hipMemsetAsync(c->dump.p, 0xff, (size_t)words * 4, c->stream));
        p.dump = (uint32_t*)c->dump.p;
        p.dump_rows = c->dump_rows;
        p.redo_mask = nullptr;
        p.src64.coef = nullptr;
        c->pend_redo.armed = false;
        c->dump_dims[0] = n_cand; c->dump_dims[1] = ns; c->dump_dims[2] = n_hyp; c->dump_dims[3] = c->dump_rows;
        c->dump_ncont_n = 0;
    }
    if (launch_lmeds<0>(c, p, step_knots, chunk, &c->last_lmeds_cap, &c->last_lmeds_chunk)) return 1;
    c->pend_redo.p = p;
    if (c->batch_n) {
        c->pend_redo.armed = false;
        c->redo_dirty = true;
        if (launch_plan_sum(c, p.frame_cost, n_cand, ns, bslot, bn)) return 1;
        c->pend.rows = n_cand;
        return 0;
    }
    if (launch_plan_sum(c, p.frame_cost, n_cand, ns)) return 1;
    size_t end = 0;
    if (queue_sums_to_host(c, n_cand, 0, &c->pend.off_chunk, &end)) return 1;
    c->pend.off_flags = end;
    RS_HIP(hipMemcpyAsync((char*)c->pinned + end, c->flags.p, 4, hipMemcpyDeviceToHost, c->stream));
    c->pend.rows = n_cand;
    c->pend.frame_costs = want_frame_costs != 0;
    c->pend.best_h = want_best_h != 0;
    return 0;
}

int rship_presync_batch_begin(rship_ctx* c, uint32_t n, uint32_t n_cand) {
    if (!n) {
        c->batch_n = c->batch_next = 0;
        c->pend = rship_ctx::Pend{};
        return 0;
    }
    if (n > 4096) return set_err(c, "presync batch: 1 .. 4096 sweeps");
    c->batch_n = n;
    c->batch_next = 0;
    c->batch_rows = n_cand;
    c->pend = rship_ctx::Pend{};
    return 0;
}
int rship_presync_batch_collect(rship_ctx* c, uint32_t n_cand, double* win_costs, double* chunk_costs, uint32_t* flags) {
    DeviceGuard dev_guard(c);
    const uint32_t n = c->batch_n;
    if (!n) return set_err(c, "presync batch: none open");
    c->batch_n = 0;
    if (flags) memset(flags, 0, (size_t)n * 4);
    if (!c->pend.rows) {
        if (win_costs) memset(win_costs, 0, (size_t)n * n_cand * (c->plan_wins ? c->plan_wins : 1) * 8);
        if (chunk_costs) memset(chunk_costs, 0, (size_t)n * n_cand * c->plan_chunks * 8);
        return 0;
    }
    if (c->batch_next != n || n_cand != c->batch_rows) return set_err(c, "presync batch: fewer sweeps were enqueued than the batch was opened for");
    const size_t cs = (size_t)n_cand * (c->plan_chunks + 1), ws = (size_t)n_cand * c->plan_wins;
    const size_t b_win = n * ws * 8, b_chunk = n * cs * 8, b_flags = (size_t)n * 4;
    if (ensure_pinned(c, b_win + b_chunk + b_flags + 64)) return 1;
    char* h = (char*)c->pinned;
    RS_HIP(hipMemcpyAsync(h, c->win_out.p, b_win, hipMemcpyDeviceToHost, c->stream));
    RS_HIP(hipMemcpyAsync(h + b_win, c->chunk_out.p, b_chunk, hipMemcpyDeviceToHost, c->stream));
    RS_HIP(hipMemcpyAsync(h + b_win + b_chunk, c->flags.p, b_flags, hipMemcpyDeviceToHost, c->stream));
    if (sync_stream(c)) return 1;
    if (win_costs) memcpy(win_costs, h, b_win);
    if (chunk_costs) {
        const double* src = (const double*)(h + b_win);
        for (uint32_t b = 0; b < n; ++b) memcpy(chunk_costs + (size_t)b * n_cand * c->plan_chunks, src + (size_t)b * cs, (size_t)n_cand * c->plan_chunks * 8);
    }
    if (flags) memcpy(flags, h + b_win + b_chunk, b_flags);
    c->pend.rows = 0;
    return 0;
}

int rship_presync_collect(rship_ctx* c, uint32_t n_cand, double* win_costs, double* chunk_costs, uint32_t* flags,
                          double* frame_costs, int32_t* best_h) {
    DeviceGuard dev_guard(c);
    if (flags) *flags = 0;
    if (!c->pend.rows) {
        if (win_costs) memset(win_costs, 0, (size_t)n_cand * (c->plan_wins ? c->plan_wins : 1) * 8);
        if (chunk_costs) memset(chunk_costs, 0, (size_t)n_cand * c->plan_chunks * 8);
        return 0;
    }
    if (n_cand != c->pend.rows) return set_err(c, "presync_collect: candidate count differs from the enqueue");
    if (sync_stream(c)) return 1;
    const uint32_t ns = c->n_sel;
    {
        uint32_t fl = 0;
        memcpy(&fl, (char*)c->pinned + c->pend.off_flags, 4);
        if ((fl & RSHIP_NEAR_STATIC) && c->pend_redo.armed) {
            c->redo_dirty = true;
            LmedsParams p = c->pend_redo.p;
            const size_t pad = ((size_t)n_cand + 1) / 2 * 2;
            if (!c->pend_redo.uploaded) {
                if (ensure(c, c->redo_delays, pad * 4 + (size_t)n_cand * 8)) return 1;
                RS_HIP(hipMemcpyAsync(c->redo_delays.p, c->h_kd64r.data(), (size_t)n_cand * 4, hipMemcpyHostToDevice, c->stream));
                RS_HIP(hipMemcpyAsync((char*)c->redo_delays.p + pad * 4, c->h_fd64r.data(), (size_t)n_cand * 8, hipMemcpyHostToDevice, c->stream));
            }
            p.kd64 = (const int32_t*)c->redo_delays.p;
            p.fd64 = (const double*)((const char*)c->redo_delays.p + pad * 4);
            if (launch_lmeds_redo(c, p, c->pend_redo.step_knots, c->pend_redo.chunk)) return 1;
            c->redo_dirty = false;
            c->near_launches += 1;
            if (launch_plan_sum(c, p.frame_cost, n_cand, ns)) return 1;
            size_t end = 0;
            if (queue_sums_to_host(c, n_cand, 0, &c->pend.off_chunk, &end)) return 1;
            c->pend.off_flags = end;
            RS_HIP(hipMemcpyAsync((char*)c->pinned + end, c->flags.p, 4, hipMemcpyDeviceToHost, c->stream));
            if (sync_stream(c)) return 1;
        }
        c->pend_redo.armed = false;
    }
    if (win_costs) memcpy(win_costs, c->pinned, (size_t)n_cand * c->plan_wins * 8);
    if (chunk_costs) memcpy(chunk_costs, (char*)c->pinned + c->pend.off_chunk, (size_t)n_cand * c->plan_chunks * 8);
    if (flags) memcpy(flags, (char*)c->pinned + c->pend.off_flags, 4);
    if (frame_costs) RS_HIP(hipMemcpy(frame_costs, c->frame_cost.p, (size_t)n_cand * ns * 8, hipMemcpyDeviceToHost));
    if (best_h && c->pend.best_h) RS_HIP(hipMemcpy(best_h, c->best_h.p, (size_t)n_cand * ns * 4, hipMemcpyDeviceToHost));
    c->pend.rows = 0;
    return 0;
}

namespace {
int fill_motion(rship_ctx* c, Motion64Params& p) {
    p.scratch = nullptr;
    p.scratch_rows = 0;
    p.scratch0 = 0;
    if (c->cls_off[5] != c->cls_off[6]) {
        const uint32_t rows = big_rows(c->cls_max_n[5]);
        if (ensure(c, c->mo_scratch, (size_t)(c->cls_off[6] - c->cls_off[5]) * 3 * rows * 8)) return 1;
        p.scratch = (double*)c->mo_scratch.p;
        p.scratch_rows = rows;
    }
    p.rays = rays64_of(c);
    p.frames = (const FrameRec*)c->frames.p;
    p.sel = (const uint32_t*)c->sel.p;
    p.n_sel = c->n_sel;
    p.coef = (const d4*)c->coef64.p;
    p.n_knots = (int)c->n_knots;
    p.kd = (const int32_t*)c->kd64.p;
    p.fd = c->d_fd64;
    p.grp = c->n_grp > 1 ? (const uint32_t*)c->grp.p : nullptr;
    p.M = (double*)c->M.p;
    p.k = (double*)c->k.p;
    p.reeval = c->lbfgs_reeval;
    p.max_iters = 200;
    p.init_h = (int32_t*)c->init_h.p;
    p.seed = c->init_seed;
    p.stream_base = c->init_stream;
    p.stream_stride = c->init_stride;
    p.simple_k = 0;
    p.evals_out = (uint32_t*)c->mo_evals.p;
    p.order = (const uint32_t*)c->mo_order.p;
    return 0;
}

int prepare_order(rship_ctx* c, const std::vector<std::pair<uint32_t, uint32_t>>& ranges) {
    if (!c->mo_identity && ranges != c->mo_ranges) {
        RS_HIP(hipStreamSynchronize(c->stream));
        RS_HIP(hipMemcpy(c->mo_order.p, c->h_cls_slots.data(), (size_t)(c->n_sel + 1) * 4, hipMemcpyHostToDevice));
    }
    c->mo_identity = false;
    c->mo_ranges = ranges;
    return 0;
}
int prepare_order_all(rship_ctx* c) { return prepare_order(c, {{0u, c->n_sel}}); }
}

int rship_init_motion(rship_ctx* c, const int32_t* kd, const float* fd, const int32_t* kd64, const double* fd64, uint32_t n_hyp, uint32_t stream,
                      uint32_t stream_stride, uint64_t seed) {
    DeviceGuard dev_guard(c);
    if (check_ready(c)) return 1;
    if (upload_delays(c, kd, fd, c->n_grp) || ensure(c, c->flags, 16)) return 1;
    RS_HIP(hipMemsetAsync(c->flags.p, 0, 16, c->stream));
    LmedsParams p{};
    p.rays_a = (const f4*)c->rays_a.p;
    p.rays_b = (const f4*)c->rays_b.p;
    p.frames = (const FrameRec*)c->frames.p;
    p.sel = (const uint32_t*)c->sel.p;
    p.n_sel = c->n_sel;
    p.coef = (const f4*)c->coef.p;
    p.n_knots = (int)c->n_knots;
    p.kd = (const int32_t*)c->kd.p;
    p.fd = c->d_fd;
    p.n_cand = 1;
    p.chunk = 1;
    p.n_chunks = 1;
    p.n_hyp = n_hyp;
    p.stream_base = stream;
    p.stream_stride = stream_stride;
    p.seed = seed;
    p.grp = c->n_grp > 1 ? (const uint32_t*)c->grp.p : nullptr;
    p.n_grp = c->n_grp;
    p.best_h = (int32_t*)c->init_h.p;
    p.flags = (uint32_t*)c->flags.p;
    if (!c->no_fp64_rows && c->rays64.p && c->coef64.p) {
        const uint32_t ng = c->n_grp;
        const size_t pad = ((size_t)ng + 1) / 2 * 2;
        if (ensure(c, c->init_delays64, pad * 4 + (size_t)ng * 8) || ensure_redo_count(c)) return 1;
        c->h_init64.assign(pad + 2 * (size_t)ng, 0u);
        for (uint32_t i = 0; i < ng; ++i) {
            const int32_t k = kd64 ? kd64[i] : kd[i];
            const double f = fd64 ? fd64[i] : (double)fd[i];
            memcpy(&c->h_init64[i], &k, 4);
            memcpy(&c->h_init64[pad + 2 * (size_t)i], &f, 8);
        }
        RS_HIP(hipMemcpyAsync(c->init_delays64.p, c->h_init64.data(), pad * 4 + (size_t)ng * 8, hipMemcpyHostToDevice, c->stream));
        p.src64 = Rows64Src{rays64_of(c), (const d4*)c->coef64.p, (int)c->n_knots};
        p.kd64 = (const int32_t*)c->init_delays64.p;
        p.fd64 = (const double*)((const char*)c->init_delays64.p + pad * 4);
        p.redo_count = (unsigned long long*)c->redo_count.p;
    }
#if RSSYNC_TEST_VARIANTS
    if (c->dump_on) {
        const uint32_t ns = c->n_sel;
        const uint64_t words = (uint64_t)ns * n_hyp * c->dump_rows;
        if (words > ((uint64_t)3 << 30) / 4) return set_err(c, "debug_residuals: more than 3 GB of residuals: search fewer frames per call");
        if (ensure(c, c->dump, (size_t)words * 4) || ensure(c, c->dump_ncont, (size_t)ns * 4)) return 1;
        RS_HIP(hipMemsetAsync(c->dump.p, 0xff, (size_t)words * 4, c->stream));
        RS_HIP(hipMemsetAsync(c->dump_ncont.p, 0, (size_t)ns * 4, c->stream));
        p.dump = (uint32_t*)c->dump.p;
        p.dump_rows = c->dump_rows;
        p.dump_ncont = (uint32_t*)c->dump_ncont.p;
        p.src64.coef = nullptr;
        c->dump_dims[0] = 1; c->dump_dims[1] = ns; c->dump_dims[2] = n_hyp; c->dump_dims[3] = c->dump_rows;
        c->dump_ncont_n = ns;
    }
#endif
    if (launch_lmeds<1>(c, p, 0.0, 1u, &c->last_init_cap, nullptr)) return 1;
    c->init_pending = true;
    c->init_seed = seed;
    c->init_stream = stream;
    c->init_stride = stream_stride;
    return 0;
}

int rship_finish_init(rship_ctx* c, const int32_t* kd, const double* fd) {
    DeviceGuard dev_guard(c);
    if (check_ready(c)) return 1;
    if (!c->init_pending) return 0;
    if (upload_delays64(c, kd, fd, c->n_grp)) return 1;
    Motion64Params p{};
    if (fill_motion(c, p)) return 1;
    p.max_iters = 0;
    if (prepare_order_all(c) || launch_motion64(c, p)) return 1;
    c->init_pending = false;
    return sync_stream(c);
}

int rship_init_k_simple(rship_ctx* c, const int32_t* kd, const double* fd) {
    DeviceGuard dev_guard(c);
    if (check_ready(c)) return 1;
    if (upload_delays64(c, kd, fd, c->n_grp)) return 1;
    Motion64Params p{};
    if (fill_motion(c, p)) return 1;
    p.init_h = nullptr;
    p.simple_k = 1;
    if (prepare_order_all(c) || launch_motion64(c, p)) return 1;
    return sync_stream(c);
}

int rship_opt_motion_detail(rship_ctx* c, const int32_t* kd, const double* fd, uint32_t* per_frame, uint32_t cap) {
    DeviceGuard dev_guard(c);
    if (check_ready(c)) return 1;
    if (cap < c->n_sel) return set_err(c, "opt_motion_detail: output too small");
    TempBuf d;
    if (ensure(c, d, (size_t)c->n_sel * 8 + 8)) return 1;
    RS_HIP(hipMemsetAsync(d.p, 0, (size_t)c->n_sel * 8 + 8, c->stream));
    if (upload_delays64(c, kd, fd, c->n_grp)) return 1;
    Motion64Params p{};
    if (fill_motion(c, p)) return 1;
    p.per_frame = (uint32_t*)d.p;
    int rc = prepare_order_all(c) || launch_motion64(c, p);
    c->init_pending = false;
    hipError_t e = hipStreamSynchronize(c->stream);
    prof_collect(c);
    if (!rc && e == hipSuccess) e = hipMemcpy(per_frame, d.p, (size_t)c->n_sel * 8, hipMemcpyDeviceToHost);
    if (rc) return 1;
    if (e != hipSuccess) return set_err(c, "opt_motion_detail", e);
    return 0;
}

int rship_opt_motion(rship_ctx* c, const int32_t* kd, const double* fd, uint64_t* stats) {
    DeviceGuard dev_guard(c);
    if (check_ready(c)) return 1;
    if (stats) {
        if (ensure(c, c->stats, 32)) return 1;
        RS_HIP(hipMemsetAsync(c->stats.p, 0, 32, c->stream));
    }
    if (upload_delays64(c, kd, fd, c->n_grp)) return 1;
    Motion64Params p{};
    if (fill_motion(c, p)) return 1;
    p.stats = stats ? (unsigned long long*)c->stats.p : nullptr;
    if (prepare_order_all(c) || launch_motion64(c, p)) return 1;
    c->init_pending = false;
    if (stats) {
        if (ensure_pinned(c, 32)) return 1;
        RS_HIP(hipMemcpyAsync(c->pinned, c->stats.p, 24, hipMemcpyDeviceToHost, c->stream));
        if (sync_stream(c)) return 1;
        memcpy(stats, c->pinned, 24);
        return 0;
    }
    return 0;
}

int rship_loss_enqueue(rship_ctx* c, const int32_t* kd, const double* fd, uint32_t n_delays, int want_grad, uint32_t flags) {
    DeviceGuard dev_guard(c);
    c->pend = rship_ctx::Pend{};
    if (!c->n_knots) return set_err(c, "no gyro spline uploaded");
    const uint32_t ns = c->n_sel, ng = c->n_grp;
    if (!n_delays || !ns) return 0;
    const bool simple = (flags & RSHIP_LOSS_SIMPLIFIED) != 0;
    if (c->init_pending && !simple) return set_err(c, "loss: the motion initialisation has not been finished");
    if (upload_delays64(c, kd, fd, (size_t)n_delays * ng)) return 1;
    if (ensure(c, c->part, (size_t)n_delays * ns * 16)) return 1;
    Loss64Params p{};
    p.rays = rays64_of(c);
    p.frames = (const FrameRec*)c->frames.p;
    p.sel = (const uint32_t*)c->sel.p;
    p.n_sel = ns;
    p.coef = (const d4*)c->coef64.p;
    p.n_knots = (int)c->n_knots;
    p.fs = c->fs;
    p.kd = (const int32_t*)c->kd64.p;
    p.fd = c->d_fd64;
    p.n_delays = n_delays;
    p.grp = ng > 1 ? (const uint32_t*)c->grp.p : nullptr;
    p.n_grp = ng;
    p.M = (const double*)c->M.p;
    p.k = (const double*)c->k.p;
    p.part_loss = (double*)c->part.p;
    p.part_grad = p.part_loss + (size_t)n_delays * ns;
    int rc;
    if (simple) rc = want_grad ? launch_loss64<true, true>(c, p) : launch_loss64<false, true>(c, p);
    else rc = want_grad ? launch_loss64<true, false>(c, p) : launch_loss64<false, false>(c, p);
    if (rc) return 1;
    const uint32_t rows = want_grad ? 2 * n_delays : n_delays;
    if (launch_plan_sum(c, p.part_loss, rows, ns)) return 1;
    size_t end = 0;
    if (queue_sums_to_host(c, rows, 0, &c->pend.off_chunk, &end)) return 1;
    c->pend.rows = rows;
    c->pend.grad = want_grad != 0;
    return 0;
}

int rship_loss_collect(rship_ctx* c, uint32_t n_delays, double* win_loss, double* win_grad, double* chunk_loss,
                       double* chunk_grad) {
    DeviceGuard dev_guard(c);
    const size_t wn = (size_t)n_delays * (c->plan_wins ? c->plan_wins : 1), cn = (size_t)n_delays * c->plan_chunks;
    if (!c->pend.rows) {
        if (win_loss) memset(win_loss, 0, wn * 8);
        if (win_grad) memset(win_grad, 0, wn * 8);
        if (chunk_loss) memset(chunk_loss, 0, cn * 8);
        if (chunk_grad) memset(chunk_grad, 0, cn * 8);
        return 0;
    }
    if (n_delays * (c->pend.grad ? 2u : 1u) != c->pend.rows) return set_err(c, "loss_collect: row count differs from the enqueue");
    if (sync_stream(c)) return 1;
    const char* base = (const char*)c->pinned;
    if (win_loss) memcpy(win_loss, base, wn * 8);
    if (win_grad && c->pend.grad) memcpy(win_grad, base + wn * 8, wn * 8);
    if (chunk_loss) memcpy(chunk_loss, base + c->pend.off_chunk, cn * 8);
    if (chunk_grad && c->pend.grad) memcpy(chunk_grad, base + c->pend.off_chunk + cn * 8, cn * 8);
    c->pend.rows = 0;
    return 0;
}

static uint32_t loop_groups(const rship_ctx* c, uint32_t n_win) {
    uint32_t g = 4;
    if (const char* s = std::getenv("RSSYNC_LOOP_STREAMS")) { const int v = atoi(s); if (v >= 1 && v <= 16) g = (uint32_t)v; }
    if (c->prof) g = 1;
    const uint32_t by_size = n_win / 8;
    if (g > by_size) g = by_size;
    return g < 1 ? 1 : g;
}

static int sync_run_body(rship_ctx* c, const double* d0, int max_outer, double search_center, double search_radius,
                         int simplified, double* d_out, int32_t* iters, double* trace);
int rship_sync_run(rship_ctx* c, const double* d0, int max_outer, double search_center, double search_radius,
                   int simplified, double* d_out, int32_t* iters, double* trace) {
    const int rc = sync_run_body(c, d0, max_outer, search_center, search_radius, simplified, d_out, iters, trace);
    if (rc && c->rccl_comm) rccl_abort_comm(c);
    return rc;
}
static int sync_run_body(rship_ctx* c, const double* d0, int max_outer, double search_center, double search_radius,
                         int simplified, double* d_out, int32_t* iters, double* trace) {
    DeviceGuard dev_guard(c);
    const bool ranked = c->rccl_comm != nullptr || c->loop_xchg != nullptr;
    if (!c->n_knots) return set_err(c, "no gyro spline uploaded");
    if (!ranked && check_ready(c)) return 1;
    const uint32_t W = c->n_grp, ns = c->n_sel;
    if (c->plan_wins != W || c->plan_has_idx || c->plan_len != ns) return set_err(c, "sync_run: the plan must be the selection's groups");
    if (max_outer <= 0) return set_err(c, "sync_run: no iterations");
    if (c->h_grp_off.size() != (size_t)W + 1) return set_err(c, "sync_run: no selection");
    const uint32_t G = ranked ? 1u : loop_groups(c, W);
    rccl_allreduce_fn allreduce = nullptr;
    if (ranked && !c->loop_xchg && !(allreduce = (rccl_allreduce_fn)rccl_sym(c, "ncclAllReduce"))) return 1;
    std::vector<double> xbuf;
    c->loop_exchanges = 0;
    int nf_fixed = 0;
    if (const char* e = std::getenv("RSSYNC_LOOP_FIRST_TRIALS")) { const int v = atoi(e); if (v >= 1 && v <= kMaxBt) nf_fixed = v; }
    int nf_floor = (!ranked && c->max_n >= 1024u) ? 1 : kHalfBt;
    if (const char* e = std::getenv("RSSYNC_LOOP_TRIALS_FLOOR")) { const int v = atoi(e); if (v >= 1 && v <= kMaxBt) nf_floor = v; }
    const int max_launch = 2 * max_outer;
    size_t off = 0;
    auto take = [&](size_t bytes) { size_t o = off; off += (bytes + 255) / 256 * 256; return o; };
    const size_t o_win = take(W * sizeof(SyncWin));
    const size_t o_mokd = take(W * 4), o_mofd = take(W * 8), o_lgkd = take(W * 4), o_lgfd = take(W * 8);
    const size_t o_trkd = take((size_t)kMaxBt * W * 4), o_trfd = take((size_t)kMaxBt * W * 8);
    const size_t nact_stride = ((size_t)max_launch * 4 + 255) / 256 * 256;
    const size_t o_nact = take((size_t)G * nact_stride);
    const size_t o_trace = take((size_t)W * max_outer * 48);
    const size_t o_tmp = take((size_t)W * 2 * kMaxBt * (c->plan_max_chunks + 1) * 8);
    const size_t o_ext = take((size_t)2 * kMaxBt * W * 8);
    if (ensure(c, c->loop_state, off)) return 1;
    char* base = (char*)c->loop_state.p;
    if (ensure(c, c->part, (size_t)2 * kMaxBt * (ns + 1) * 8)) return 1;
    while (c->loop_streams.size() < G) {
        hipStream_t st = nullptr;
        RS_HIP(hipStreamCreateWithFlags(&st, hipStreamNonBlocking));
        c->loop_streams.push_back(st);
    }
    if (!c->loop_ready) RS_HIP(hipEventCreateWithFlags(&c->loop_ready, hipEventDisableTiming));

    std::vector<SyncWin> hw(W);
    for (uint32_t w = 0; w < W; ++w) {
        hw[w] = SyncWin{};
        hw[w].d = d0[w];
        hw[w].active = 1;
        hw[w].hit = -1;
        hw[w].nf = nf_fixed ? nf_fixed : nf_floor;
    }
    RS_HIP(hipMemcpyAsync(base + o_win, hw.data(), W * sizeof(SyncWin), hipMemcpyHostToDevice, c->stream));
    RS_HIP(hipMemsetAsync(base + o_nact, 0, (size_t)G * nact_stride, c->stream));

    SyncLoopParams lp{};
    lp.win = (SyncWin*)(base + o_win);
    lp.n_win = W;
    lp.part = (const double*)c->part.p;
    lp.n_sel = ns;
    lp.chunk_off = (const uint32_t*)c->plan_chunk_off.p;
    lp.win_chunk_off = (const uint32_t*)c->plan_win_off.p;
    lp.chunk_tmp = (double*)(base + o_tmp);
    lp.chunk_stride = c->plan_max_chunks + 1;
    lp.mo_kd = (int32_t*)(base + o_mokd); lp.mo_fd = (double*)(base + o_mofd);
    lp.lg_kd = (int32_t*)(base + o_lgkd); lp.lg_fd = (double*)(base + o_lgfd);
    lp.tr_kd = (int32_t*)(base + o_trkd); lp.tr_fd = (double*)(base + o_trfd);
    lp.fs = c->fs;
    {
        double t = 1e-3;
        for (int i = 0; i <= kMaxBt; ++i) { lp.ts[i] = t; t *= .1; }
    }
    lp.c_armijo = 2e-4;
    lp.delay_b = .3;
    lp.search_center = search_center;
    lp.search_radius = search_radius;
    lp.max_outer = max_outer;
    lp.nf_fixed = nf_fixed;
    lp.nf_floor = nf_floor;
    lp.trace = (double*)(base + o_trace);
    lp.ext_sums = ranked ? (double*)(base + o_ext) : nullptr;

    Motion64Params mp{};
    if (fill_motion(c, mp)) return 1;
    mp.kd = lp.mo_kd;
    mp.fd = lp.mo_fd;
    Loss64Params qp{};
    qp.rays = rays64_of(c);
    qp.frames = (const FrameRec*)c->frames.p;
    qp.sel = (const uint32_t*)c->sel.p;
    qp.n_sel = ns;
    qp.coef = (const d4*)c->coef64.p;
    qp.n_knots = (int)c->n_knots;
    qp.fs = c->fs;
    qp.grp = W > 1 ? (const uint32_t*)c->grp.p : nullptr;
    qp.n_grp = W;
    qp.M = (const double*)c->M.p;
    qp.k = (const double*)c->k.p;
    qp.part_loss = (double*)c->part.p;

    struct Group {
        uint32_t w0, w1, s0, s1;
        hipStream_t st;
        int* n_active;
        int* h_nact;
        int it = 0;
        bool done = false;
    };
    std::vector<Group> groups(G);
    if (ensure_pinned(c, (size_t)G * nact_stride + 64)) return 1;
    {
        uint32_t w = 0;
        for (uint32_t g = 0; g < G; ++g) {
            Group& gr = groups[g];
            gr.w0 = w;
            const uint64_t target = (uint64_t)ns * (g + 1) / G;
            while (w < W && (g + 1 == G || c->h_grp_off[w + 1] <= target || w == gr.w0)) ++w;
            if (g + 1 == G) w = W;
            gr.w1 = w;
            gr.s0 = c->h_grp_off[gr.w0];
            gr.s1 = c->h_grp_off[gr.w1];
            gr.st = G == 1 ? c->stream : c->loop_streams[g];
            gr.n_active = (int*)(base + o_nact + (size_t)g * nact_stride);
            gr.h_nact = (int*)((char*)c->pinned + (size_t)g * nact_stride);
            gr.done = gr.w1 == gr.w0;
        }
    }
    {
        std::vector<std::pair<uint32_t, uint32_t>> ranges;
        for (const Group& gr : groups)
            if (gr.s1 > gr.s0)
                for (const ClassRange& r : class_ranges(c, gr.s0, gr.s1 - gr.s0)) ranges.emplace_back(r.pos0, r.count);
        if (prepare_order(c, ranges)) return 1;
    }
    if (G > 1) {
        RS_HIP(hipEventRecord(c->loop_ready, c->stream));
        for (Group& gr : groups) RS_HIP(hipStreamWaitEvent(gr.st, c->loop_ready, 0));
    }
    auto enqueue_iteration = [&](Group& gr) -> int {
        SyncLoopParams l = lp;
        l.win0 = gr.w0; l.win1 = gr.w1;
        l.n_active = gr.n_active;
        l.it = gr.it;
        const uint32_t nw = gr.w1 - gr.w0, cnt = gr.s1 - gr.s0;
        const dim3 ctl_block(nw > 64 ? 64 : kBlock);
        Loss64Params q = qp;
        auto loss_launch = [&](bool grad) -> int {
            if (simplified) return grad ? launch_loss64<true, true>(c, q, gr.st, gr.s0, cnt) : launch_loss64<false, true>(c, q, gr.st, gr.s0, cnt);
            return grad ? launch_loss64<true, false>(c, q, gr.st, gr.s0, cnt) : launch_loss64<false, false>(c, q, gr.st, gr.s0, cnt);
        };
        if (gr.it == 0) {
            hipLaunchKernelGGL(sync_begin_kernel, dim3((nw + 63) / 64), dim3(64), 0, gr.st, l);
            RS_HIP(hipGetLastError());
        }
        if (!simplified && cnt) {
            if (launch_motion64(c, mp, gr.st, gr.s0, cnt)) return 1;
        }
        q.kd = l.lg_kd; q.fd = l.lg_fd; q.n_delays = 1;
        q.part_grad = q.part_loss + (size_t)ns;
        if (cnt && loss_launch(true)) return 1;
        l.rows = 2;
        auto exchange = [&](uint32_t rows) -> int {
            if (!ranked) return 0;
            hipLaunchKernelGGL(sync_sums_kernel, dim3(nw), ctl_block, 0, gr.st, l);
            RS_HIP(hipGetLastError());
            c->loop_exchanges += 1;
            if (c->loop_xchg) {
                xbuf.resize((size_t)rows * W);
                RS_HIP(hipMemcpyAsync(xbuf.data(), l.ext_sums, xbuf.size() * 8, hipMemcpyDeviceToHost, gr.st));
                RS_HIP(hipStreamSynchronize(gr.st));
                const int rc = c->loop_xchg(c->loop_xchg_user, xbuf.data(), xbuf.size());
                if (rc) return set_err(c, "sync_run: the loop's host exchange failed (" + std::to_string(rc) + ")");
                RS_HIP(hipMemcpyAsync(l.ext_sums, xbuf.data(), xbuf.size() * 8, hipMemcpyHostToDevice, gr.st));
                RS_HIP(hipStreamSynchronize(gr.st));
                return 0;
            }
            const int rc = allreduce(l.ext_sums, l.ext_sums, (size_t)rows * W,  8,  0, c->rccl_comm, gr.st);
            if (rc) return set_err(c, "rccl: ncclAllReduce failed (" + std::to_string(rc) + ")");
            return 0;
        };
        if (exchange(2)) return 1;
        {
            ProfScope ps(c, RSHIP_K_REDUCE);
            hipLaunchKernelGGL(sync_grad_kernel, dim3(nw), ctl_block, 0, gr.st, l);
        }
        q.kd = l.tr_kd; q.fd = l.tr_fd; q.n_delays = kMaxBt;
        q.part_grad = nullptr;
        l.rows = kMaxBt;
        if (cnt && loss_launch(false)) return 1;
        if (exchange(kMaxBt)) return 1;
        {
            ProfScope ps(c, RSHIP_K_REDUCE);
            hipLaunchKernelGGL(sync_step_kernel, dim3(nw), ctl_block, 0, gr.st, l);
        }
        RS_HIP(hipGetLastError());
        gr.it += 1;
        return 0;
    };

    const int kLook = 8;
    auto run_group = [&](Group& gr) -> int {
        DeviceGuard guard(c);
        while (!gr.done) {
            const int later = !ranked ? kLook / 2 : (c->loop_xchg ? 1 : 2);
            const int first = (ranked && c->loop_xchg) ? 1 : kLook;
            const int until = std::min(max_launch, gr.it + (gr.it == 0 ? first : later));
            while (gr.it < until)
                if (enqueue_iteration(gr)) return 1;
            RS_HIP(hipMemcpyAsync(gr.h_nact, gr.n_active, (size_t)gr.it * 4, hipMemcpyDeviceToHost, gr.st));
            RS_HIP(hipStreamSynchronize(gr.st));
            gr.done = gr.h_nact[gr.it - 1] == 0 || gr.it >= max_launch;
        }
        return 0;
    };
    {
        std::vector<std::thread> workers;
        std::vector<int> rc(G, 0);
        for (uint32_t g = 1; g < G; ++g) workers.emplace_back([&, g] { rc[g] = run_group(groups[g]); });
        rc[0] = run_group(groups[0]);
        for (std::thread& t : workers) t.join();
        for (uint32_t g = 0; g < G; ++g)
            if (rc[g]) return 1;
    }
    int it_max = 0;
    for (const Group& gr : groups) it_max = std::max(it_max, gr.it);
    it_max = std::min(it_max, max_outer);
    c->init_pending = false;
    if (G == 1) prof_collect(c);
    const size_t tr_bytes = (size_t)it_max * W * 48, win_bytes = W * sizeof(SyncWin);
    if (ensure_pinned(c, tr_bytes + win_bytes + 64)) return 1;
    RS_HIP(hipMemcpyAsync(c->pinned, base + o_win, win_bytes, hipMemcpyDeviceToHost, c->stream));
    RS_HIP(hipMemcpyAsync((char*)c->pinned + win_bytes, base + o_trace, tr_bytes, hipMemcpyDeviceToHost, c->stream));
    if (sync_stream(c)) return 1;
    memcpy(hw.data(), c->pinned, win_bytes);
    const double* tr = (const double*)((const char*)c->pinned + win_bytes);
    for (uint32_t w = 0; w < W; ++w) {
        d_out[w] = hw[w].d;
        iters[w] = hw[w].iters;
        for (int k = 0; k < hw[w].iters; ++k) memcpy(trace + ((size_t)w * max_outer + k) * 6, tr + ((size_t)k * W + w) * 6, 48);
    }
    return 0;
}

namespace {
size_t exec_region_bytes(rship_ctx* c) {
    uint32_t search_cap = 0;
    if (c->cls_off[1] != c->cls_off[0]) search_cap = plan_lmeds_window<1>(c, 0, 0.0, 1u).cap;
    size_t region = rs::exec_region_for(c->cls_cap64[0], compact_of(c, 0), search_cap);
    if (c->n_sel != c->cls_off[1] - c->cls_off[0]) region = std::max(region, (size_t)16 * 1024);
    for (int k = 1; k < 5; ++k)
        if (c->cls_off[k + 1] != c->cls_off[k]) {
            const WinPlan wp = plan_lmeds_window<1>(c, k, 0.0, 1u);
            region = std::max(region, (size_t)(wp.cap ? wp.cap : (uint32_t)kWinMax) * 64u);
        }
    return region;
}
}
int rship_exec_supported(rship_ctx* c) {
    if (c->force_big || !c->n_sel || c->n_sel >= (1u << 24)) return 0;
    for (uint32_t i : c->h_sel)
        if (c->h_frame_n[i] < 2) return 0;
    if (c->max_n > c->one_wave_max && c->max_n > c->exec_big_max) return 0;
    if (c->cls_off[5] != c->cls_off[4]) return 0;
    if ((uint64_t)(c->n_sel - (c->cls_off[1] - c->cls_off[0])) * c->exec_big_share > c->n_sel) return 0;
    return exec_region_bytes(c) <= 48u * 1024u ? 1 : 0;
}

int rship_sync_exec(rship_ctx* c, const double* d0, int repeats, uint32_t stream_first, uint32_t stream_stride, uint64_t seed,
                    int max_outer, double search_center, double search_radius, double* d_out, double* cost, int32_t* iters,
                    double* trace, uint32_t trace_rows) {
    DeviceGuard dev_guard(c);
    if (check_ready(c)) return 1;
    const uint32_t W = c->n_grp, ns = c->n_sel;
    if (!rship_exec_supported(c)) return set_err(c, "sync_exec: this selection is not for the executor (RSSYNC_FORCE_BIG, a frame of fewer than 2 tracks, a search window beyond a wave's LDS)");
    if (c->plan_wins != W || c->plan_has_idx || c->plan_len != ns) return set_err(c, "sync_exec: the plan must be the selection's groups");
    if (max_outer <= 0 || repeats < 1 || repeats > kExecMaxCalls) return set_err(c, "sync_exec: bad iteration or call count");
    if (trace_rows < (uint32_t)repeats * (uint32_t)max_outer) return set_err(c, "sync_exec: trace too small");
    if (c->h_grp_off.size() != (size_t)W + 1) return set_err(c, "sync_exec: no selection");
    for (uint32_t w = 0; w < W; ++w)
        if (c->h_grp_off[w + 1] == c->h_grp_off[w]) return set_err(c, "sync_exec: a window without frames");
    int nf_fixed = 0;
    if (const char* e = std::getenv("RSSYNC_LOOP_FIRST_TRIALS")) { const int v = atoi(e); if (v >= 1 && v <= kMaxBt) nf_fixed = v; }
    int n_cu = 256;
    (void)hipDeviceGetAttribute(&n_cu, hipDeviceAttributeMultiprocessorCount, c->device);
    const uint32_t exec_rpt = (uint32_t)small_rpt(c->cls_max_n[0]);
    const size_t region = exec_region_bytes(c);
    if (region < (size_t)kExecStage * sizeof(double)) return set_err(c, "sync_exec: the wave's LDS region is smaller than the decisions' staging area");
    const bool compact = compact_of(c, 0);
    const uint32_t cap64 = (uint32_t)(region / (compact ? 64u : 128u));
    const bool with_big = ns != c->cls_off[1] - c->cls_off[0];
    uint32_t per_cu = 8;
    {
        int occ = 0;
        uint32_t fixed_lds = 0;
        hipError_t e = hipSuccess;
#define RS_EXEC_OCC(R)                                                                                                                  \
    case R:                                                                                                                             \
        fixed_lds = with_big ? static_lds_of(sync_exec_kernel<R, true>) : static_lds_of(sync_exec_kernel<R, false>);                    \
        e = with_big ? hipOccupancyMaxActiveBlocksPerMultiprocessor(&occ, sync_exec_kernel<R, true>, 64, region)                        \
                     : hipOccupancyMaxActiveBlocksPerMultiprocessor(&occ, sync_exec_kernel<R, false>, 64, region);                      \
        break;
        switch (exec_rpt) {
            RS_EXEC_OCC(1)
            RS_EXEC_OCC(2)
            RS_EXEC_OCC(3)
            RS_EXEC_OCC(4)
            default: RS_EXEC_OCC(8)
        }
#undef RS_EXEC_OCC
        if (e != hipSuccess) { (void)hipGetLastError(); occ = 0; }
        const size_t per_wave = fixed_lds + region + 512;
        const uint32_t fit = (uint32_t)((size_t)c->lds_per_cu / per_wave);
        if (fit < per_cu) per_cu = fit < 1 ? 1 : fit;
        if (occ >= 1 && (uint32_t)occ < per_cu) per_cu = (uint32_t)occ;
    }
    uint32_t waves = (uint32_t)n_cu * per_cu;
    if (waves > ns) waves = ns;
    uint32_t q_cap = 256, q_shift = 8;
    while (q_cap < 4 * (ns + 9 * (ns - (c->cls_off[1] - c->cls_off[0])) + waves)) { q_cap *= 2; ++q_shift; }
    size_t off = 0;
    auto take = [&](size_t bytes) { size_t o = off; off += (bytes + 255) / 256 * 256; return o; };
    const size_t o_win = take(W * sizeof(ExecWin));
    const size_t o_inkd = take(W * 4), o_infd = take(W * 4), o_stream = take(W * 4);
    const size_t o_inkd64 = take(W * 4), o_infd64 = take(W * 8);
    const size_t o_mokd = take(W * 4), o_mofd = take(W * 8), o_lgkd = take(W * 4), o_lgfd = take(W * 8);
    const size_t o_trkd = take((size_t)kMaxBt * W * 4), o_trfd = take((size_t)kMaxBt * W * 8);
    constexpr size_t kCtlStride = 128;
    const size_t o_q = take((size_t)q_cap * 8), o_ctl = take(4 * kCtlStride);
    const size_t o_trace = take((size_t)W * trace_rows * 48);
    const uint32_t n_big = ns - (c->cls_off[1] - c->cls_off[0]);
    uint32_t big_rows_n = 0;
    for (int k = 1; k < kNumClasses; ++k) big_rows_n = std::max(big_rows_n, c->cls_max_n[k]);
    big_rows_n = big_rows(big_rows_n);
    const size_t o_info = take(n_big ? (size_t)ns * 4 : 0), o_big = take(n_big ? sizeof(ExecBig) : 0);
    const size_t o_wboff = take(n_big ? (size_t)(W + 1) * 4 : 0), o_blist = take(n_big ? (size_t)n_big * 4 : 0);
    if (ensure(c, c->loop_state, off) || ensure(c, c->part, (size_t)2 * kMaxBt * ns * 8) || ensure(c, c->flags, 16)) return 1;
    if (n_big && (ensure(c, c->big_scratch, (size_t)n_big * big_rows_n * kExecBigFloats * 4) ||
                  ensure(c, c->mo_scratch, (size_t)n_big * 3 * big_rows_n * 8)))
        return 1;
    char* base = (char*)c->loop_state.p;
    std::vector<uint32_t> slot_info, win_big_off, big_list;
    if (n_big) {
        slot_info.assign(ns, 0u);
        uint32_t entry = 0;
        for (int k = 1; k < kNumClasses; ++k)
            for (uint32_t e = c->cls_off[k]; e < c->cls_off[k + 1]; ++e) slot_info[c->h_cls_slots[e]] = ((entry++ + 1u) << 3) | (uint32_t)k;
        win_big_off.assign(W + 1, 0u);
        for (uint32_t w = 0; w < W; ++w) {
            for (uint32_t j = c->h_grp_off[w]; j < c->h_grp_off[w + 1]; ++j)
                if (slot_info[j]) big_list.push_back(j);
            win_big_off[w + 1] = (uint32_t)big_list.size();
        }
        RS_HIP(hipMemcpyAsync(base + o_info, slot_info.data(), (size_t)ns * 4, hipMemcpyHostToDevice, c->stream));
        RS_HIP(hipMemcpyAsync(base + o_wboff, win_big_off.data(), (size_t)(W + 1) * 4, hipMemcpyHostToDevice, c->stream));
        RS_HIP(hipMemcpyAsync(base + o_blist, big_list.data(), (size_t)n_big * 4, hipMemcpyHostToDevice, c->stream));
    }

    std::vector<ExecWin> hw(W);
    std::vector<int32_t> in_kd(W), in_kd64(W);
    std::vector<float> in_fd(W);
    std::vector<double> in_fd64(W);
    std::vector<uint32_t> streams(W);
    std::vector<unsigned long long> queue(q_cap, 0ull);
    const double kClamp = (double)(1 << 29);
    for (uint32_t w = 0; w < W; ++w) {
        ExecWin& e = hw[w];
        e = ExecWin{};
        e.s.d = d0[w];
        e.s.active = 1;
        e.s.hit = -1;
        e.s.nf = nf_fixed ? nf_fixed : kHalfBt;
        e.s.x0 = d0[w] - .3 * 0.0;
        e.slot0 = c->h_grp_off[w];
        e.n_slots = c->h_grp_off[w + 1] - c->h_grp_off[w];
        e.phase = kPhInit;
        e.remaining = e.n_slots;
        streams[w] = stream_first + w * stream_stride;
        const double D = d0[w] * c->fs;
        in_kd64[w] = 0; in_fd64[w] = 0.0;
        if (std::isfinite(D)) {
            const double fl64 = std::floor(D);
            if (fl64 > kClamp) in_kd64[w] = (int32_t)kClamp;
            else if (fl64 < -kClamp) in_kd64[w] = (int32_t)-kClamp;
            else { in_kd64[w] = (int32_t)fl64; in_fd64[w] = D - fl64; }
        }
        if (!std::isfinite(D)) { in_kd[w] = 0; in_fd[w] = 0.f; }
        else {
            double fl = std::floor(D);
            float f = (float)(D - fl);
            if (f >= 1.0f) { f = 0.f; fl += 1.0; }
            fl = std::min(std::max(fl, -kClamp), kClamp);
            in_kd[w] = (int32_t)fl;
            in_fd[w] = f;
        }
    }
    for (uint32_t j = 0; j < ns; ++j) queue[j] = (1ull << 32) | ((unsigned long long)kPhInit << 24) | j;
    uint32_t ctl[4 * kCtlStride / 4] = {};
    ctl[kCtlStride / 4] = ns;
    RS_HIP(hipMemcpyAsync(base + o_win, hw.data(), W * sizeof(ExecWin), hipMemcpyHostToDevice, c->stream));
    RS_HIP(hipMemcpyAsync(base + o_inkd, in_kd.data(), W * 4, hipMemcpyHostToDevice, c->stream));
    RS_HIP(hipMemcpyAsync(base + o_infd, in_fd.data(), W * 4, hipMemcpyHostToDevice, c->stream));
    RS_HIP(hipMemcpyAsync(base + o_inkd64, in_kd64.data(), W * 4, hipMemcpyHostToDevice, c->stream));
    RS_HIP(hipMemcpyAsync(base + o_infd64, in_fd64.data(), W * 8, hipMemcpyHostToDevice, c->stream));
    RS_HIP(hipMemcpyAsync(base + o_stream, streams.data(), W * 4, hipMemcpyHostToDevice, c->stream));
    RS_HIP(hipMemcpyAsync(base + o_q, queue.data(), (size_t)q_cap * 8, hipMemcpyHostToDevice, c->stream));
    RS_HIP(hipMemcpyAsync(base + o_ctl, ctl, sizeof(ctl), hipMemcpyHostToDevice, c->stream));

    ExecParams ep{};
    {
        double t = 1e-3;
        for (int i = 0; i <= kMaxBt; ++i) { ep.lp.ts[i] = t; t *= .1; }
    }
    ep.lp.fs = c->fs;
    ep.lp.c_armijo = 2e-4;
    ep.lp.delay_b = .3;
    ep.lp.search_center = search_center;
    ep.lp.search_radius = search_radius;
    ep.lp.max_outer = max_outer;
    ep.lp.nf_fixed = nf_fixed;
    ep.lp.nf_floor = kHalfBt;
    ep.win = (ExecWin*)(base + o_win);
    ep.n_win = W;
    ep.n_sel = ns;
    ep.grp = (const uint32_t*)c->grp.p;
    ep.in_kd = (int32_t*)(base + o_inkd); ep.in_fd = (float*)(base + o_infd);
    ep.win_stream = (uint32_t*)(base + o_stream);
    ep.mo_kd = (int32_t*)(base + o_mokd); ep.mo_fd = (double*)(base + o_mofd);
    ep.lg_kd = (int32_t*)(base + o_lgkd); ep.lg_fd = (double*)(base + o_lgfd);
    ep.tr_kd = (int32_t*)(base + o_trkd); ep.tr_fd = (double*)(base + o_trfd);
    ep.part = (double*)c->part.p;
    ep.chunk_off = (const uint32_t*)c->plan_chunk_off.p;
    ep.win_chunk_off = (const uint32_t*)c->plan_win_off.p;
    ep.trace = (double*)(base + o_trace);
    ep.trace_rows = trace_rows;
    ep.stream_first = stream_first;
    ep.stream_stride = stream_stride;
    ep.repeats = repeats;
    ep.q = (unsigned long long*)(base + o_q);
    ep.q_mask = q_cap - 1;
    ep.q_shift = q_shift;
    ep.q_head = (uint32_t*)(base + o_ctl);
    ep.q_tail = (uint32_t*)(base + o_ctl + kCtlStride);
    ep.done = (uint32_t*)(base + o_ctl + 2 * kCtlStride);
    ep.abort_flag = (uint32_t*)(base + o_ctl + 3 * kCtlStride);
    double wd_s = 5.0;
    if (const char* s = std::getenv("RSSYNC_EXEC_WATCHDOG_S")) { const double v = atof(s); if (v > 0.0 && v < 600.0) wd_s = v; }
    ep.watchdog_ticks = (unsigned long long)(wd_s * 1e8);
    ep.init.rays_a = (const f4*)c->rays_a.p;
    ep.init.rays_b = (const f4*)c->rays_b.p;
    ep.init.frames = (const FrameRec*)c->frames.p;
    ep.init.sel = (const uint32_t*)c->sel.p;
    ep.init.n_sel = ns;
    ep.init.slots = nullptr;
    ep.init.n_slots = ns;
    ep.init.coef = (const f4*)c->coef.p;
    ep.init.n_knots = (int)c->n_knots;
    ep.init.kd = ep.in_kd;
    ep.init.fd = ep.in_fd;
    ep.init.n_cand = 1; ep.init.chunk = 1; ep.init.n_chunks = 1;
    ep.init.n_hyp = 200;
    ep.init.seed = seed;
    ep.init.win_stream = ep.win_stream;
    ep.init.grp = ep.grp;
    ep.init.n_grp = W;
    ep.init.best_h = (int32_t*)c->init_h.p;
    ep.init.flags = (uint32_t*)c->flags.p;
    if (!c->no_fp64_rows && c->rays64.p && c->coef64.p) {
        if (ensure_redo_count(c)) return 1;
        ep.init.src64 = Rows64Src{rays64_of(c), (const d4*)c->coef64.p, (int)c->n_knots};
        ep.init.kd64 = (const int32_t*)(base + o_inkd64);
        ep.init.fd64 = (const double*)(base + o_infd64);
        ep.init.redo_count = (unsigned long long*)c->redo_count.p;
    }
    {
        const WinPlan wp_init = plan_lmeds_window<1>(c, 0, 0.0, 1u);
        ep.init.win_cap = wp_init.cap ? wp_init.cap : (uint32_t)kWinMax;
        ep.init.win_whole_pair = (wp_init.cap && !wp_init.whole_pair) ? 0u : 1u;
        if ((size_t)ep.init.win_cap * 64u > region) return set_err(c, "sync_exec: the search's window does not fit the wave's LDS region");
    }
    ExecBig hb{};
    ep.big = nullptr;
    if (n_big) {
        hb.slot_info = (const uint32_t*)(base + o_info);
        hb.win_big_off = (const uint32_t*)(base + o_wboff);
        hb.big_list = (const uint32_t*)(base + o_blist);
        hb.big_tile = (float*)c->big_scratch.p;
        hb.big_P = (double*)c->mo_scratch.p;
        hb.big_rows = big_rows_n;
        hb.init_whole = 0;
// ... 1936 lines not shown
```

Baseline: 137.9 billion.

## Cut per-call host overhead: batch setup uploads, fuse copies, fold sort into step kernel

Replaces many small per-call memcpy/memset operations with a pinned upload ring and a single multi-job setup kernel. Host-side copies of selection and plan data are cached so unchanged inputs skip re-uploading, and redundant flag memsets are skipped. The flag readback is merged into the sums transfer, and the window/trace readback becomes one copy. The motion-order sort is folded into extra blocks of sync_step_kernel, and n_active zeroing moves into sync_begin_kernel. This removes launch and transfer latency at the cost of more state-tracking complexity and a risk of stale-cache bugs.

```diff
diff --git a/rs-sync_amd/csrc/kernels/setup.hpp b/rs-sync_amd/csrc/kernels/setup.hpp
--- /dev/null
+++ b/rs-sync_amd/csrc/kernels/setup.hpp
@@ -0,0 +1,43 @@
+#pragma once
+
+#include <stdint.h>
+
+namespace {
+
+enum : uint32_t {
+    kSetupCopy = 0,
+    kSetupFill = 1,
+    kSetupIota = 2,
+};
+constexpr int kSetupMaxJobs = 12;
+constexpr int kSetupBlock = 256;
+constexpr uint32_t kSetupMaxGrid = 64;
+
+struct SetupJob {
+    uint32_t* dst;
+    const uint32_t* src;
+    uint32_t count;
+    uint32_t value;
+    uint32_t kind;
+    uint32_t pad_;
+};
+struct SetupParams {
+    SetupJob job[kSetupMaxJobs];
+    uint32_t n_jobs;
+};
+
+__global__ __launch_bounds__(kSetupBlock) void select_setup_kernel(SetupParams p) {
+    const uint32_t t0 = blockIdx.x * kSetupBlock + threadIdx.x, stride = gridDim.x * kSetupBlock;
+    for (uint32_t j = 0; j < p.n_jobs; ++j) {
+        const SetupJob jb = p.job[j];
+        if (jb.kind == kSetupCopy) {
+            for (uint32_t i = t0; i < jb.count; i += stride) jb.dst[i] = jb.src[i];
+        } else if (jb.kind == kSetupFill) {
+            for (uint32_t i = t0; i < jb.count; i += stride) jb.dst[i] = jb.value;
+        } else {
+            for (uint32_t i = t0; i < jb.count; i += stride) jb.dst[i] = i;
+        }
+    }
+}
+
+}
diff --git a/rs-sync_amd/csrc/kernels/support.hpp b/rs-sync_amd/csrc/kernels/support.hpp
--- a/rs-sync_amd/csrc/kernels/support.hpp
+++ b/rs-sync_amd/csrc/kernels/support.hpp
@@ -6,8 +6,11 @@
                                                          const uint32_t* __restrict__ idx,
                                                          const uint32_t* __restrict__ chunk_off, uint32_t n_chunks,
                                                          const uint32_t* __restrict__ win_chunk_off, uint32_t n_win,
-                                                         double* __restrict__ chunk_out, double* __restrict__ win_out) {
+                                                         double* __restrict__ chunk_out, double* __restrict__ win_out,
+                                                         const uint32_t* __restrict__ flags_in) {
     const uint32_t r = blockIdx.x / n_win, w = blockIdx.x % n_win;
+    if (flags_in && blockIdx.x == 0 && threadIdx.x == 0)
+        *reinterpret_cast<uint32_t*>(chunk_out + (size_t)(gridDim.x / n_win) * n_chunks) = *flags_in;
     const uint32_t c0 = win_chunk_off[w], c1 = win_chunk_off[w + 1];
     const double* row = in + (size_t)r * n_cols;
     double* cout = chunk_out + (size_t)r * n_chunks;
diff --git a/rs-sync_amd/csrc/kernels/sync64.hpp b/rs-sync_amd/csrc/kernels/sync64.hpp
--- a/rs-sync_amd/csrc/kernels/sync64.hpp
+++ b/rs-sync_amd/csrc/kernels/sync64.hpp
@@ -568,9 +568,8 @@
                                p.scratch0 + blockIdx.x);
 }
 
-__global__ __launch_bounds__(1024) void motion_order_kernel(const uint32_t* __restrict__ evals, const uint32_t* __restrict__ list,
-                                                            uint32_t* __restrict__ order, uint32_t pos0, uint32_t count) {
-    __shared__ uint32_t s_bin[256];
+__device__ __forceinline__ void motion_order_block(const uint32_t* __restrict__ evals, const uint32_t* __restrict__ list,
+                                                   uint32_t* __restrict__ order, uint32_t pos0, uint32_t count, uint32_t* s_bin) {
     for (uint32_t b = threadIdx.x; b < 256; b += blockDim.x) s_bin[b] = 0;
     __syncthreads();
     for (uint32_t i = threadIdx.x; i < count; i += blockDim.x) {
@@ -593,6 +592,11 @@
         const uint32_t pos = atomicAdd(&s_bin[e < 255u ? e : 255u], 1u);
         order[pos0 + pos] = s;
     }
+}
+__global__ __launch_bounds__(1024) void motion_order_kernel(const uint32_t* __restrict__ evals, const uint32_t* __restrict__ list,
+                                                            uint32_t* __restrict__ order, uint32_t pos0, uint32_t count) {
+    __shared__ uint32_t s_bin[256];
+    motion_order_block(evals, list, order, pos0, count, s_bin);
 }
 
 struct Debug64Params {
diff --git a/rs-sync_amd/csrc/kernels/syncloop.hpp b/rs-sync_amd/csrc/kernels/syncloop.hpp
--- a/rs-sync_amd/csrc/kernels/syncloop.hpp
+++ b/rs-sync_amd/csrc/kernels/syncloop.hpp
@@ -13,6 +13,8 @@
     int nf;
     int hit_prev;
 };
+
+constexpr int kMaxOrderRanges = 6;
 
 struct SyncLoopParams {
     SyncWin* win;
@@ -35,7 +37,13 @@
     int nf_floor;
     double* ext_sums;
     int* n_active;
+    int max_launch;
     double* trace;
+    const uint32_t* mo_evals;
+    const uint32_t* mo_list;
+    uint32_t* mo_order;
+    uint32_t mo_ranges;
+    uint32_t mo_pos0[kMaxOrderRanges], mo_count[kMaxOrderRanges];
 };
 
 
@@ -114,6 +122,8 @@
 
 __global__ __launch_bounds__(64) void sync_begin_kernel(SyncLoopParams p) {
 #pragma clang fp contract(off)
+    if (blockIdx.x == 0)
+        for (int i = threadIdx.x; i < p.max_launch; i += 64) p.n_active[i] = 0;
     const uint32_t w = p.win0 + blockIdx.x * 64 + threadIdx.x;
     if (w >= p.win1) return;
     SyncWin& s = p.win[w];
@@ -232,6 +242,11 @@
 #pragma clang fp contract(off)
     __shared__ double s_tot[2 * kMaxBt];
     __shared__ double s_stage[kStageDoubles];
+    if (blockIdx.x >= p.win1 - p.win0) {
+        const uint32_t j = blockIdx.x - (p.win1 - p.win0);
+        motion_order_block(p.mo_evals, p.mo_list, p.mo_order, p.mo_pos0[j], p.mo_count[j], reinterpret_cast<uint32_t*>(s_stage));
+        return;
+    }
     const uint32_t w = blockIdx.x + p.win0;
     decision_sums(p, w, s_tot, s_stage);
     if (threadIdx.x != 0) return;
diff --git a/rs-sync_amd/csrc/rssync_kernels.hip b/rs-sync_amd/csrc/rssync_kernels.hip
--- a/rs-sync_amd/csrc/rssync_kernels.hip
+++ b/rs-sync_amd/csrc/rssync_kernels.hip
@@ -68,6 +68,7 @@
 #include "kernels/colorzoom.hpp"
 #include "kernels/infill.hpp"
 #include "kernels/colorinfill.hpp"
+#include "kernels/setup.hpp"
 
 
 struct DevBuf {
@@ -84,6 +85,8 @@
 };
 
 constexpr int kNumClasses = 6;
+static_assert(kMaxOrderRanges >= kNumClasses, "a motion launch has one range per size class");
+constexpr size_t kFlagsHead = 20;
 
 struct rship_ctx {
     int device = 0;
@@ -169,7 +172,6 @@
     uint32_t exec_last[4] = {0, 0, 0, 0};
     std::vector<uint32_t> h_frame_n;
     std::vector<uint32_t> h_sel;
-    std::vector<uint32_t> h_delays, h_delays64;
     const float* d_fd = nullptr;
     DevBuf kd64;
     const double* d_fd64 = nullptr;
@@ -186,6 +188,16 @@
     DevBuf dump, dump_ncont;
     bool dump_on = false;
     uint32_t dump_rows = 0, dump_dims[4] = {0, 0, 0, 0}, dump_ncont_n = 0;
+    struct UpSlot { void* h = nullptr; size_t cap = 0; hipEvent_t done = nullptr; bool busy = false; };
+    static constexpr int kUpSlots = 4;
+    UpSlot up_ring[kUpSlots];
+    uint32_t up_next = 0;
+    DevBuf setup_blob;
+    std::vector<uint32_t> h_res_sel;
+    bool res_single = false, sel_valid = false;
+    bool flags_clean = false;
+    std::vector<uint32_t> h_plan_idx, h_plan_chunk_off, h_plan_win_off;
+    bool plan_valid = false;
     DevBuf kd, frame_cost, best_h, costs, part, flags, stats;
     void* pinned = nullptr;
     size_t pinned_cap = 0;
@@ -236,6 +248,61 @@
     size_t want = bytes + bytes / 4 + 4096;
     RS_HIP(hipHostMalloc(&c->pinned, want, hipHostMallocDefault));
     c->pinned_cap = want;
+    return 0;
+}
+
+int ring_acquire(rship_ctx* c, size_t bytes, rship_ctx::UpSlot** out) {
+    rship_ctx::UpSlot& s = c->up_ring[c->up_next];
+    c->up_next = (c->up_next + 1) % rship_ctx::kUpSlots;
+    if (s.busy) {
+        RS_HIP(hipEventSynchronize(s.done));
+        s.busy = false;
+    }
+    if (!s.done) RS_HIP(hipEventCreateWithFlags(&s.done, hipEventDisableTiming));
+    if (bytes > s.cap) {
+        if (s.h) RS_HIP(hipHostFree(s.h));
+        s.h = nullptr;
+        s.cap = 0;
+        const size_t want = bytes + bytes / 4 + 256;
+        RS_HIP(hipHostMalloc(&s.h, want, hipHostMallocDefault));
+        s.cap = want;
+    }
+    *out = &s;
+    return 0;
+}
+int ring_upload(rship_ctx* c, rship_ctx::UpSlot* s, size_t bytes, void* dst = nullptr) {
+    if (!bytes) return 0;
+    if (!dst) {
+        if (ensure(c, c->setup_blob, bytes)) return 1;
+        dst = c->setup_blob.p;
+    }
+    RS_HIP(hipMemcpyAsync(dst, s->h, bytes, hipMemcpyHostToDevice, c->stream));
+    RS_HIP(hipEventRecord(s->done, c->stream));
+    s->busy = true;
+    return 0;
+}
+struct SetupList {
+    SetupParams p{};
+    bool overflow = false;
+    void add(uint32_t kind, void* dst, const void* src, size_t count, uint32_t value = 0) {
+        if (!count) return;
+        if (p.n_jobs == (uint32_t)kSetupMaxJobs) { overflow = true; return; }
+        SetupJob& j = p.job[p.n_jobs++];
+        j.dst = (uint32_t*)dst;
+        j.src = (const uint32_t*)src;
+        j.count = (uint32_t)count;
+        j.value = value;
+        j.kind = kind;
+    }
+};
+int launch_setup(rship_ctx* c, const SetupList& l) {
+    if (l.overflow) return set_err(c, "call set-up: too many jobs");
+    if (!l.p.n_jobs) return 0;
+    uint32_t most = 0;
+    for (uint32_t j = 0; j < l.p.n_jobs; ++j) most = std::max(most, l.p.job[j].count);
+    const uint32_t grid = std::min(kSetupMaxGrid, (most + kSetupBlock - 1) / kSetupBlock);
+    hipLaunchKernelGGL(select_setup_kernel, dim3(grid), dim3(kSetupBlock), 0, c->stream, l.p);
+    RS_HIP(hipGetLastError());
     return 0;
 }
 
@@ -712,7 +779,8 @@
 
 constexpr uint32_t kOrderMinSlots = 512;
 
-int launch_motion64(rship_ctx* c, const Motion64Params& p_in, hipStream_t st = nullptr, uint32_t slot0 = 0, uint32_t count = 0) {
+int launch_motion64(rship_ctx* c, const Motion64Params& p_in, hipStream_t st = nullptr, uint32_t slot0 = 0, uint32_t count = 0,
+                    std::vector<std::pair<uint32_t, uint32_t>>* sort_later = nullptr) {
     if (!st) st = c->stream;
     ProfScope ps(c, RSHIP_K_MOTION);
     for (const ClassRange& r : class_ranges(c, slot0, count)) {
@@ -743,6 +811,10 @@
         }
         RS_HIP(hipGetLastError());
         if (p.evals_out && p.order && c->mo_order.p && p.max_iters > 0 && !p.simple_k && cnt >= kOrderMinSlots) {
+            if (sort_later) {
+                sort_later->emplace_back(r.pos0, cnt);
+                continue;
+            }
             hipLaunchKernelGGL(motion_order_kernel, dim3(1), dim3(1024), 0, st, (const uint32_t*)p.evals_out, (const uint32_t*)c->cls_slots.p,
                                (uint32_t*)c->mo_order.p, r.pos0, cnt);
             RS_HIP(hipGetLastError());
@@ -751,25 +823,25 @@
     return 0;
 }
 
-int launch_plan_sum(rship_ctx* c, const double* in, uint32_t rows, uint32_t cols, uint32_t slot = 0, uint32_t n_slots = 1) {
+int launch_plan_sum(rship_ctx* c, const double* in, uint32_t rows, uint32_t cols, const uint32_t* flags = nullptr, bool batch = false, uint32_t slot = 0, uint32_t n_slots = 1) {
     if (!c->plan_wins) return set_err(c, "no reduction plan set");
     const size_t cs = (size_t)rows * (c->plan_chunks + 1), ws = (size_t)rows * c->plan_wins;
-    if (n_slots > 1 && (c->chunk_out.cap < cs * n_slots * 8 || c->win_out.cap < ws * n_slots * 8)) return set_err(c, "plan sum: the batch's buffers were not sized");
-    if (n_slots == 1 && (ensure(c, c->chunk_out, cs * 8) || ensure(c, c->win_out, ws * 8))) return 1;
+    if (batch && (c->chunk_out.cap < cs * n_slots * 8 || c->win_out.cap < ws * n_slots * 8)) return set_err(c, "plan sum: the batch's buffers were not sized");
+    if (!batch && ensure(c, c->win_out, (ws + cs) * 8)) return 1;
+    double* const win = (double*)c->win_out.p + (batch ? ws * slot : 0);
+    double* const chunk = batch ? (double*)c->chunk_out.p + cs * slot : win + ws;
     ProfScope ps(c, RSHIP_K_REDUCE);
     hipLaunchKernelGGL(plan_sum_kernel, dim3(rows * c->plan_wins), dim3(64), 0, c->stream, in, cols,
                        c->plan_has_idx ? (const uint32_t*)c->plan_idx.p : nullptr, (const uint32_t*)c->plan_chunk_off.p,
-                       c->plan_chunks, (const uint32_t*)c->plan_win_off.p, c->plan_wins, (double*)c->chunk_out.p + cs * slot,
-                       (double*)c->win_out.p + ws * slot);
+                       c->plan_chunks, (const uint32_t*)c->plan_win_off.p, c->plan_wins, chunk, win, batch ? nullptr : flags);
     RS_HIP(hipGetLastError());
     return 0;
 }
 
-int queue_sums_to_host(rship_ctx* c, uint32_t rows, size_t at, size_t* off_chunk, size_t* end) {
+int queue_sums_to_host(rship_ctx* c, uint32_t rows, size_t at, size_t* off_chunk, size_t* end, bool with_flags = false) {
     const size_t wb = (size_t)rows * c->plan_wins * 8, cb = (size_t)rows * c->plan_chunks * 8;
     if (ensure_pinned(c, at + wb + cb + 64)) return 1;
-    RS_HIP(hipMemcpyAsync((char*)c->pinned + at, c->win_out.p, wb, hipMemcpyDeviceToHost, c->stream));
-    if (cb) RS_HIP(hipMemcpyAsync((char*)c->pinned + at + wb, c->chunk_out.p, cb, hipMemcpyDeviceToHost, c->stream));
+    RS_HIP(hipMemcpyAsync((char*)c->pinned + at, c->win_out.p, wb + cb + (with_flags ? 4 : 0), hipMemcpyDeviceToHost, c->stream));
     *off_chunk = at + wb;
     *end = at + wb + cb;
     return 0;
@@ -791,20 +863,23 @@
 
 int upload_delays(rship_ctx* c, const int32_t* kd, const float* fd, size_t n) {
     if (ensure(c, c->kd, n * 8)) return 1;
-    c->h_delays.resize(2 * n);
-    memcpy(c->h_delays.data(), kd, n * 4);
-    memcpy(c->h_delays.data() + n, fd, n * 4);
-    RS_HIP(hipMemcpyAsync(c->kd.p, c->h_delays.data(), n * 8, hipMemcpyHostToDevice, c->stream));
+    rship_ctx::UpSlot* slot = nullptr;
+    if (ring_acquire(c, n * 8, &slot)) return 1;
+    memcpy(slot->h, kd, n * 4);
+    memcpy((char*)slot->h + n * 4, fd, n * 4);
+    if (ring_upload(c, slot, n * 8, c->kd.p)) return 1;
     c->d_fd = (const float*)((const int32_t*)c->kd.p + n);
     return 0;
 }
 int upload_delays64(rship_ctx* c, const int32_t* kd, const double* fd, size_t n) {
     const size_t pad = (n + 1) / 2 * 2;
     if (ensure(c, c->kd64, pad * 4 + n * 8)) return 1;
-    c->h_delays64.resize(pad + 2 * n);
-    memcpy(c->h_delays64.data(), kd, n * 4);
-    memcpy(c->h_delays64.data() + pad, fd, n * 8);
-    RS_HIP(hipMemcpyAsync(c->kd64.p, c->h_delays64.data(), pad * 4 + n * 8, hipMemcpyHostToDevice, c->stream));
+    rship_ctx::UpSlot* slot = nullptr;
+    if (ring_acquire(c, pad * 4 + n * 8, &slot)) return 1;
+    if (pad != n) ((uint32_t*)slot->h)[n] = 0;
+    memcpy(slot->h, kd, n * 4);
+    memcpy((char*)slot->h + pad * 4, fd, n * 8);
+    if (ring_upload(c, slot, pad * 4 + n * 8, c->kd64.p)) return 1;
     c->d_fd64 = (const double*)((const int32_t*)c->kd64.p + pad);
     return 0;
 }
@@ -948,10 +1023,14 @@
                       &c->trk_slot[0], &c->trk_slot[1], &c->trk_out, &c->ftr_cells, &c->ftr_out,
                       &c->rect_rays, &c->rect_slot[0], &c->rect_slot[1], &c->rect_times, &c->rect_count, &c->rect_tmp,
                       &c->stab_weights, &c->stab_targets, &c->stab_zooms, &c->stab_cover, &c->rect_rays_c,
-                      &c->limit_goal, &c->limit_out, &c->limit_rays};
+                      &c->limit_goal, &c->limit_out, &c->limit_rays, &c->setup_blob};
     for (DevBuf* b : bufs)
         if (b->p) (void)hipFree(b->p);
     if (c->pinned) (void)hipHostFree(c->pinned);
+    for (rship_ctx::UpSlot& s : c->up_ring) {
+        if (s.h) (void)hipHostFree(s.h);
+        if (s.done) (void)hipEventDestroy(s.done);
+    }
     for (hipStream_t st : c->loop_streams) (void)hipStreamDestroy(st);
     if (c->loop_ready) (void)hipEventDestroy(c->loop_ready);
     if (c->copy_done) (void)hipEventDestroy(c->copy_done);
@@ -1502,63 +1581,98 @@
         if (idx[i] >= c->n_frames) return set_err(c, "select: frame index out of range");
     if (n_grp < 1) n_grp = 1;
     if (grp_off && (grp_off[0] != 0 || grp_off[n_grp] != n)) return set_err(c, "select: bad group offsets");
+    const void* const held[] = {c->sel.p, c->grp.p, c->grp_off.p, c->cls_slots.p, c->mo_order.p};
+    bool was_valid = c->sel_valid;
     if (ensure(c, c->sel, (size_t)n * 4 + 4) || ensure(c, c->grp, (size_t)n * 4 + 4) ||
         ensure(c, c->grp_off, (size_t)(n_grp + 1) * 4))
         return 1;
     if (ensure(c, c->M, (size_t)n * 24 + 24) || ensure(c, c->k, (size_t)n * 8 + 8) || ensure(c, c->init_h, (size_t)n * 4 + 4)) return 1;
     if (ensure(c, c->mo_evals, (size_t)n * 4 + 4) || ensure(c, c->mo_order, (size_t)n * 4 + 4)) return 1;
     c->init_pending = false;
-    std::vector<uint32_t> g(n, 0), off(n_grp + 1, 0);
-    if (grp_off) {
-        off.assign(grp_off, grp_off + n_grp + 1);
-        for (uint32_t w = 0; w < n_grp; ++w)
-            for (uint32_t j = off[w]; j < off[w + 1]; ++j) g[j] = w;
-    } else {
-        off[n_grp] = n;
-    }
-    if (n) {
-        RS_HIP(hipMemcpyAsync(c->sel.p, idx, (size_t)n * 4, hipMemcpyHostToDevice, c->stream));
-        RS_HIP(hipMemcpyAsync(c->grp.p, g.data(), (size_t)n * 4, hipMemcpyHostToDevice, c->stream));
-    }
-    RS_HIP(hipMemcpyAsync(c->grp_off.p, off.data(), (size_t)(n_grp + 1) * 4, hipMemcpyHostToDevice, c->stream));
-    RS_HIP(hipMemsetAsync(c->M.p, 0, (size_t)n * 24 + 24, c->stream));
-    RS_HIP(hipMemsetAsync(c->k.p, 0, (size_t)n * 8 + 8, c->stream));
-    RS_HIP(hipMemsetD32Async((hipDeviceptr_t)c->init_h.p, kInitNone, (size_t)n + 1, c->stream));
+    c->sel_valid = false;
+    std::vector<uint32_t> off(n_grp + 1, 0);
+    if (grp_off) off.assign(grp_off, grp_off + n_grp + 1);
+    else off[n_grp] = n;
+    std::vector<uint32_t> cls((size_t)n + 1, n);
+    uint32_t cls_off[kNumClasses + 1] = {}, mx[kNumClasses] = {};
+    int cls_used = 0;
     {
         std::vector<uint32_t> cnt(kNumClasses + 1, 0);
-        uint32_t mx[kNumClasses] = {};
         for (uint32_t i = 0; i < n; ++i) {
             const uint32_t fn = c->h_frame_n[idx[i]];
             const int k = class_of(c, fn);
             cnt[k + 1] += 1;
             mx[k] = std::max(mx[k], fn);
         }
-        c->cls_used = 0;
         for (int k = 0; k < kNumClasses; ++k) {
-            if (cnt[k + 1]) c->cls_used += 1;
-            c->cls_max_n[k] = mx[k];
-            c->cls_off[k] = cnt[k];
+            if (cnt[k + 1]) cls_used += 1;
+            cls_off[k] = cnt[k];
             cnt[k + 1] += cnt[k];
         }
-        c->cls_off[kNumClasses] = n;
-        c->h_cls_slots.assign((size_t)n + 1, n);
+        cls_off[kNumClasses] = n;
         uint32_t at[kNumClasses];
-        for (int k = 0; k < kNumClasses; ++k) at[k] = c->cls_off[k];
-        for (uint32_t i = 0; i < n; ++i) c->h_cls_slots[at[class_of(c, c->h_frame_n[idx[i]])]++] = i;
+        for (int k = 0; k < kNumClasses; ++k) at[k] = cls_off[k];
+        for (uint32_t i = 0; i < n; ++i) cls[at[class_of(c, c->h_frame_n[idx[i]])]++] = i;
         if (ensure(c, c->cls_slots, (size_t)n * 4 + 4)) return 1;
-        RS_HIP(hipMemcpyAsync(c->cls_slots.p, c->h_cls_slots.data(), (size_t)(n + 1) * 4, hipMemcpyHostToDevice, c->stream));
-        RS_HIP(hipMemcpyAsync(c->mo_order.p, c->h_cls_slots.data(), (size_t)(n + 1) * 4, hipMemcpyHostToDevice, c->stream));
-        RS_HIP(hipMemsetAsync(c->mo_evals.p, 0, (size_t)n * 4 + 4, c->stream));
-        c->mo_identity = true;
-        c->mo_ranges.clear();
-    }
-    RS_HIP(hipStreamSynchronize(c->stream));
+    }
+    {
+        const void* const now[] = {c->sel.p, c->grp.p, c->grp_off.p, c->cls_slots.p, c->mo_order.p};
+        for (int i = 0; i < 5; ++i) was_valid = was_valid && held[i] == now[i];
+    }
+    const bool same = was_valid && n == c->n_sel && n_grp == c->n_grp && off == c->h_grp_off && cls == c->h_cls_slots &&
+                      std::equal(idx, idx + n, c->h_sel.begin());
+    const bool prefix = !same && was_valid && n_grp == 1 && c->res_single && cls_used <= 1 && n <= c->h_res_sel.size() &&
+                        std::equal(idx, idx + n, c->h_res_sel.begin());
+    SetupList jobs;
+    if (same) {
+        jobs.add(kSetupCopy, c->mo_order.p, c->cls_slots.p, (size_t)n + 1);
+    } else if (prefix) {
+        jobs.add(kSetupFill, (uint32_t*)c->grp_off.p + 1, nullptr, 1, n);
+        jobs.add(kSetupIota, c->cls_slots.p, nullptr, (size_t)n + 1);
+        jobs.add(kSetupIota, c->mo_order.p, nullptr, (size_t)n + 1);
+    } else {
+        const size_t o_sel = 0, o_grp = n, o_off = 2 * (size_t)n, o_cls = o_off + n_grp + 1, words = o_cls + n + 1;
+        rship_ctx::UpSlot* slot = nullptr;
+        if (ring_acquire(c, words * 4, &slot)) return 1;
+        uint32_t* h = (uint32_t*)slot->h;
+        if (n) memcpy(h + o_sel, idx, (size_t)n * 4);
+        if (n) memset(h + o_grp, 0, (size_t)n * 4);
+        for (uint32_t w = 0; grp_off && w < n_grp; ++w)
+            for (uint32_t j = off[w]; j < off[w + 1]; ++j) h[o_grp + j] = w;
+        memcpy(h + o_off, off.data(), (size_t)(n_grp + 1) * 4);
+        memcpy(h + o_cls, cls.data(), (size_t)(n + 1) * 4);
+        if (ring_upload(c, slot, words * 4)) return 1;
+        const uint32_t* d = (const uint32_t*)c->setup_blob.p;
+        jobs.add(kSetupCopy, c->sel.p, d + o_sel, n);
+        jobs.add(kSetupCopy, c->grp.p, d + o_grp, n);
+        jobs.add(kSetupCopy, c->grp_off.p, d + o_off, (size_t)n_grp + 1);
+        jobs.add(kSetupCopy, c->cls_slots.p, d + o_cls, (size_t)n + 1);
+        jobs.add(kSetupCopy, c->mo_order.p, d + o_cls, (size_t)n + 1);
+        c->h_res_sel.assign(idx, idx + n);
+        c->res_single = n_grp == 1 && !grp_off;
+    }
+    jobs.add(kSetupFill, c->M.p, nullptr, ((size_t)n + 1) * 6, 0u);
+    jobs.add(kSetupFill, c->k.p, nullptr, ((size_t)n + 1) * 2, 0u);
+    jobs.add(kSetupFill, c->init_h.p, nullptr, (size_t)n + 1, (uint32_t)kInitNone);
+    jobs.add(kSetupFill, c->mo_evals.p, nullptr, (size_t)n + 1, 0u);
+    c->flags_clean = false;
+    if (ensure(c, c->flags, kFlagsHead)) return 1;
+    jobs.add(kSetupFill, c->flags.p, nullptr, kFlagsHead / 4, 0u);
+    if (launch_setup(c, jobs)) return 1;
+    c->flags_clean = true;
+    c->mo_identity = true;
+    c->mo_ranges.clear();
+    c->cls_used = cls_used;
+    for (int k = 0; k <= kNumClasses; ++k) c->cls_off[k] = cls_off[k];
+    for (int k = 0; k < kNumClasses; ++k) c->cls_max_n[k] = mx[k];
+    c->h_cls_slots.swap(cls);
     c->h_sel.assign(idx, idx + n);
     c->h_grp_off = off;
     c->n_sel = n;
     c->n_grp = n_grp;
     c->max_n = 0;
     for (int k = 0; k < kNumClasses; ++k) c->max_n = std::max(c->max_n, c->cls_max_n[k]);
+    c->sel_valid = true;
     return 0;
 }
 
@@ -1573,14 +1687,38 @@
     for (uint32_t j = 0; plan_idx && j < plan_len; ++j)
         if (plan_idx[j] >= c->n_sel) return set_err(c, "plan: slot out of range");
     if (!plan_idx && plan_len > c->n_sel) return set_err(c, "plan: slot out of range");
-    if (ensure(c, c->plan_idx, (size_t)plan_len * 4 + 4) || ensure(c, c->plan_chunk_off, (size_t)(n_chunks + 1) * 4) ||
-        ensure(c, c->plan_win_off, (size_t)(n_win + 1) * 4))
-        return 1;
-    if (plan_idx && plan_len) RS_HIP(hipMemcpyAsync(c->plan_idx.p, plan_idx, (size_t)plan_len * 4, hipMemcpyHostToDevice, c->stream));
     const uint32_t zero = 0;
-    RS_HIP(hipMemcpyAsync(c->plan_chunk_off.p, n_chunks ? chunk_off : &zero, (size_t)(n_chunks + 1) * 4, hipMemcpyHostToDevice, c->stream));
-    RS_HIP(hipMemcpyAsync(c->plan_win_off.p, win_chunk_off, (size_t)(n_win + 1) * 4, hipMemcpyHostToDevice, c->stream));
-    RS_HIP(hipStreamSynchronize(c->stream));
+    const uint32_t* coff = n_chunks ? chunk_off : &zero;
+    const bool has_idx = plan_idx != nullptr && plan_len != 0;
+    const bool same = c->plan_valid && has_idx == !c->h_plan_idx.empty() && c->h_plan_chunk_off.size() == (size_t)n_chunks + 1 &&
+                      c->h_plan_win_off.size() == (size_t)n_win + 1 && (!has_idx || c->h_plan_idx.size() == plan_len) &&
+                      std::equal(coff, coff + n_chunks + 1, c->h_plan_chunk_off.begin()) &&
+                      std::equal(win_chunk_off, win_chunk_off + n_win + 1, c->h_plan_win_off.begin()) &&
+                      (!has_idx || std::equal(plan_idx, plan_idx + plan_len, c->h_plan_idx.begin()));
+    if (!same) {
+        c->plan_valid = false;
+        if (ensure(c, c->plan_idx, (size_t)plan_len * 4 + 4) || ensure(c, c->plan_chunk_off, (size_t)(n_chunks + 1) * 4) ||
+            ensure(c, c->plan_win_off, (size_t)(n_win + 1) * 4))
+            return 1;
+        const size_t n_idx = has_idx ? plan_len : 0, o_coff = n_idx, o_woff = o_coff + n_chunks + 1, words = o_woff + n_win + 1;
+        rship_ctx::UpSlot* slot = nullptr;
+        if (ring_acquire(c, words * 4, &slot)) return 1;
+        uint32_t* h = (uint32_t*)slot->h;
+        if (n_idx) memcpy(h, plan_idx, n_idx * 4);
+        memcpy(h + o_coff, coff, (size_t)(n_chunks + 1) * 4);
+        memcpy(h + o_woff, win_chunk_off, (size_t)(n_win + 1) * 4);
+        if (ring_upload(c, slot, words * 4)) return 1;
+        const uint32_t* d = (const uint32_t*)c->setup_blob.p;
+        SetupList jobs;
+        jobs.add(kSetupCopy, c->plan_idx.p, d, n_idx);
+        jobs.add(kSetupCopy, c->plan_chunk_off.p, d + o_coff, (size_t)n_chunks + 1);
+        jobs.add(kSetupCopy, c->plan_win_off.p, d + o_woff, (size_t)n_win + 1);
+        if (launch_setup(c, jobs)) return 1;
+        c->h_plan_idx.assign(plan_idx, plan_idx + n_idx);
+        c->h_plan_chunk_off.assign(coff, coff + n_chunks + 1);
+        c->h_plan_win_off.assign(win_chunk_off, win_chunk_off + n_win + 1);
+        c->plan_valid = true;
+    }
     c->plan_has_idx = plan_idx != nullptr;
     c->plan_max_chunks = 0;
     for (uint32_t w = 0; w < n_win; ++w) c->plan_max_chunks = std::max(c->plan_max_chunks, win_chunk_off[w + 1] - win_chunk_off[w]);
@@ -1608,10 +1746,13 @@
     if (!n_cand || !ns) return 0;
     if (ensure(c, c->frame_cost, (size_t)n_cand * ns * 8)) return 1;
     if (want_best_h && ensure(c, c->best_h, (size_t)n_cand * ns * 4)) return 1;
+    const void* const flags_were = c->flags.p;
     if (ensure(c, c->flags, 16 + 4 * (size_t)bn)) return 1;
     if (bslot == 0) {
         if (upload_delays(c, kd, fd, n_cand)) return 1;
-        RS_HIP(hipMemsetAsync(c->flags.p, 0, 16 + 4 * (size_t)bn, c->stream));
+        if (!c->flags_clean || c->flags.p != flags_were || 16 + 4 * (size_t)bn > kFlagsHead)
+            RS_HIP(hipMemsetAsync(c->flags.p, 0, 16 + 4 * (size_t)bn, c->stream));
+        c->flags_clean = false;
         if (c->batch_n) {
             if (!c->plan_wins) return set_err(c, "no reduction plan set");
             if (ensure(c, c->chunk_out, (size_t)bn * n_cand * (c->plan_chunks + 1) * 8) || ensure(c, c->win_out, (size_t)bn * n_cand * c->plan_wins * 8)) return 1;
@@ -1695,15 +1836,14 @@
     if (c->batch_n) {
         c->pend_redo.armed = false;
         c->redo_dirty = true;
-        if (launch_plan_sum(c, p.frame_cost, n_cand, ns, bslot, bn)) return 1;
+        if (launch_plan_sum(c, p.frame_cost, n_cand, ns, nullptr, true, bslot, bn)) return 1;
         c->pend.rows = n_cand;
         return 0;
     }
-    if (launch_plan_sum(c, p.frame_cost, n_cand, ns)) return 1;
+    if (launch_plan_sum(c, p.frame_cost, n_cand, ns, p.flags)) return 1;
     size_t end = 0;
-    if (queue_sums_to_host(c, n_cand, 0, &c->pend.off_chunk, &end)) return 1;
+    if (queue_sums_to_host(c, n_cand, 0, &c->pend.off_chunk, &end, true)) return 1;
     c->pend.off_flags = end;
-    RS_HIP(hipMemcpyAsync((char*)c->pinned + end, c->flags.p, 4, hipMemcpyDeviceToHost, c->stream));
     c->pend.rows = n_cand;
     c->pend.frame_costs = want_frame_costs != 0;
     c->pend.best_h = want_best_h != 0;
@@ -1782,11 +1922,10 @@
             if (launch_lmeds_redo(c, p, c->pend_redo.step_knots, c->pend_redo.chunk)) return 1;
             c->redo_dirty = false;
             c->near_launches += 1;
-            if (launch_plan_sum(c, p.frame_cost, n_cand, ns)) return 1;
+            if (launch_plan_sum(c, p.frame_cost, n_cand, ns, p.flags)) return 1;
             size_t end = 0;
-            if (queue_sums_to_host(c, n_cand, 0, &c->pend.off_chunk, &end)) return 1;
+            if (queue_sums_to_host(c, n_cand, 0, &c->pend.off_chunk, &end, true)) return 1;
             c->pend.off_flags = end;
-            RS_HIP(hipMemcpyAsync((char*)c->pinned + end, c->flags.p, 4, hipMemcpyDeviceToHost, c->stream));
             if (sync_stream(c)) return 1;
         }
         c->pend_redo.armed = false;
@@ -1850,8 +1989,10 @@
                       uint32_t stream_stride, uint64_t seed) {
     DeviceGuard dev_guard(c);
     if (check_ready(c)) return 1;
+    const void* const flags_were = c->flags.p;
     if (upload_delays(c, kd, fd, c->n_grp) || ensure(c, c->flags, 16)) return 1;
-    RS_HIP(hipMemsetAsync(c->flags.p, 0, 16, c->stream));
+    if (!c->flags_clean || c->flags.p != flags_were) RS_HIP(hipMemsetAsync(c->flags.p, 0, 16, c->stream));
+    c->flags_clean = false;
     LmedsParams p{};
     p.rays_a = (const f4*)c->rays_a.p;
     p.rays_b = (const f4*)c->rays_b.p;
@@ -2085,11 +2226,11 @@
     size_t off = 0;
     auto take = [&](size_t bytes) { size_t o = off; off += (bytes + 255) / 256 * 256; return o; };
     const size_t o_win = take(W * sizeof(SyncWin));
+    const size_t o_trace = take((size_t)W * max_outer * 48);
     const size_t o_mokd = take(W * 4), o_mofd = take(W * 8), o_lgkd = take(W * 4), o_lgfd = take(W * 8);
     const size_t o_trkd = take((size_t)kMaxBt * W * 4), o_trfd = take((size_t)kMaxBt * W * 8);
     const size_t nact_stride = ((size_t)max_launch * 4 + 255) / 256 * 256;
     const size_t o_nact = take((size_t)G * nact_stride);
-    const size_t o_trace = take((size_t)W * max_outer * 48);
     const size_t o_tmp = take((size_t)W * 2 * kMaxBt * (c->plan_max_chunks + 1) * 8);
     const size_t o_ext = take((size_t)2 * kMaxBt * W * 8);
     if (ensure(c, c->loop_state, off)) return 1;
@@ -2110,8 +2251,12 @@
         hw[w].hit = -1;
         hw[w].nf = nf_fixed ? nf_fixed : nf_floor;
     }
-    RS_HIP(hipMemcpyAsync(base + o_win, hw.data(), W * sizeof(SyncWin), hipMemcpyHostToDevice, c->stream));
-    RS_HIP(hipMemsetAsync(base + o_nact, 0, (size_t)G * nact_stride, c->stream));
+    {
+        rship_ctx::UpSlot* slot = nullptr;
+        if (ring_acquire(c, W * sizeof(SyncWin), &slot)) return 1;
+        memcpy(slot->h, hw.data(), W * sizeof(SyncWin));
+        if (ring_upload(c, slot, W * sizeof(SyncWin), base + o_win)) return 1;
+    }
 
     SyncLoopParams lp{};
     lp.win = (SyncWin*)(base + o_win);
@@ -2135,6 +2280,7 @@
     lp.search_center = search_center;
     lp.search_radius = search_radius;
     lp.max_outer = max_outer;
+    lp.max_launch = max_launch;
     lp.nf_fixed = nf_fixed;
     lp.nf_floor = nf_floor;
     lp.trace = (double*)(base + o_trace);
@@ -2212,8 +2358,9 @@
             hipLaunchKernelGGL(sync_begin_kernel, dim3((nw + 63) / 64), dim3(64), 0, gr.st, l);
             RS_HIP(hipGetLastError());
         }
+        std::vector<std::pair<uint32_t, uint32_t>> sort_ranges;
         if (!simplified && cnt) {
-            if (launch_motion64(c, mp, gr.st, gr.s0, cnt)) return 1;
+            if (launch_motion64(c, mp, gr.st, gr.s0, cnt, &sort_ranges)) return 1;
         }
         q.kd = l.lg_kd; q.fd = l.lg_fd; q.n_delays = 1;
         q.part_grad = q.part_loss + (size_t)ns;
@@ -2250,7 +2397,12 @@
         if (exchange(kMaxBt)) return 1;
         {
             ProfScope ps(c, RSHIP_K_REDUCE);
-            hipLaunchKernelGGL(sync_step_kernel, dim3(nw), ctl_block, 0, gr.st, l);
+            l.mo_evals = (const uint32_t*)c->mo_evals.p;
+            l.mo_list = (const uint32_t*)c->cls_slots.p;
+            l.mo_order = (uint32_t*)c->mo_order.p;
+            l.mo_ranges = (uint32_t)sort_ranges.size();
+            for (size_t j = 0; j < sort_ranges.size(); ++j) { l.mo_pos0[j] = sort_ranges[j].first; l.mo_count[j] = sort_ranges[j].second; }
+            hipLaunchKernelGGL(sync_step_kernel, dim3(nw + l.mo_ranges), ctl_block, 0, gr.st, l);
         }
         RS_HIP(hipGetLastError());
         gr.it += 1;
@@ -2286,13 +2438,12 @@
     it_max = std::min(it_max, max_outer);
     c->init_pending = false;
     if (G == 1) prof_collect(c);
-    const size_t tr_bytes = (size_t)it_max * W * 48, win_bytes = W * sizeof(SyncWin);
-    if (ensure_pinned(c, tr_bytes + win_bytes + 64)) return 1;
-    RS_HIP(hipMemcpyAsync(c->pinned, base + o_win, win_bytes, hipMemcpyDeviceToHost, c->stream));
-    RS_HIP(hipMemcpyAsync((char*)c->pinned + win_bytes, base + o_trace, tr_bytes, hipMemcpyDeviceToHost, c->stream));
+    const size_t tr_bytes = (size_t)it_max * W * 48, win_bytes = W * sizeof(SyncWin), tr_at = o_trace - o_win;
+    if (ensure_pinned(c, tr_at + tr_bytes + 64)) return 1;
+    RS_HIP(hipMemcpyAsync(c->pinned, base + o_win, tr_at + tr_bytes, hipMemcpyDeviceToHost, c->stream));
     if (sync_stream(c)) return 1;
     memcpy(hw.data(), c->pinned, win_bytes);
-    const double* tr = (const double*)((const char*)c->pinned + win_bytes);
+    const double* tr = (const double*)((const char*)c->pinned + tr_at);
     for (uint32_t w = 0; w < W; ++w) {
         d_out[w] = hw[w].d;
         iters[w] = hw[w].iters;
@@ -2394,6 +2545,7 @@
     const size_t o_info = take(n_big ? (size_t)ns * 4 : 0), o_big = take(n_big ? sizeof(ExecBig) : 0);
     const size_t o_wboff = take(n_big ? (size_t)(W + 1) * 4 : 0), o_blist = take(n_big ? (size_t)n_big * 4 : 0);
     if (ensure(c, c->loop_state, off) || ensure(c, c->part, (size_t)2 * kMaxBt * ns * 8) || ensure(c, c->flags, 16)) return 1;
+    c->flags_clean = false;
     if (n_big && (ensure(c, c->big_scratch, (size_t)n_big * big_rows_n * kExecBigFloats * 4) ||
                   ensure(c, c->mo_scratch, (size_t)n_big * 3 * big_rows_n * 8)))
         return 1;
```

Result: no change. 138.6 billion, median of 6 (+0.5%).
